# taylorlu/voicepuppet

Hardware: AMD Instinct MI355X
Metric: PixReferNet G+D step frames/sec @256x256 bs=32 (higher is better)
Workload: dtype bf16; 1 GPU; PixReferNet G+D training step (G + 3xD + VGG16-conv3_3 perceptual + TF-Adam x2), 256x256, ngf=ndf=64, global batch 32 = 32 per GPU; global_batch=32, per_gpu_batch=32, parallelism=dp1

## Files before the change

### include/vp_hip.h

```cpp
#ifndef VP_HIP_H_
#define VP_HIP_H_

#include <stddef.h>
#include <stdint.h>

#ifdef __cplusplus
extern "C" {
#endif

enum vp_status { VP_OK = 0, VP_ERR_ARG = -1, VP_ERR_HIP = -2, VP_ERR_WORKSPACE = -3, VP_ERR_STATE = -4 };
enum vp_dtype { VP_F32 = 0, VP_BF16 = 1 };
enum vp_act { VP_ACT_NONE = 0, VP_ACT_LRELU = 1, VP_ACT_RELU = 2, VP_ACT_TANH = 3, VP_ACT_SIGMOID = 4, VP_ACT_RELU6 = 5, VP_ACT_LEAKY = 6 };

int vp_version(void);
const char* vp_last_error(void);

typedef struct vp_pixrefer_desc {
  int batch;
  int height;
  int ngf, ndf;
  int dtype;
  int training;
  float l1_weight;
  float gan_weight;
  int per_sample_bn;
  int streams;
  int d_backward_fork;
  int d_beside_vgg;
} vp_pixrefer_desc;

size_t vp_pixrefer_desc_size(void);

typedef struct vp_pixrefer vp_pixrefer_t;

size_t vp_pixrefer_param_count(const vp_pixrefer_desc* d, int which);
int vp_pixrefer_param_info(const vp_pixrefer_desc* d, int which, int index, char* name, int name_cap,
                           size_t* offset, int* ndim, int64_t shape[4]);

size_t vp_pixrefer_workspace_bytes(const vp_pixrefer_desc* d);
int vp_pixrefer_validate_plan(const vp_pixrefer_desc* d);

int vp_pixrefer_create(const vp_pixrefer_desc* d, void* workspace, size_t workspace_bytes,
                       float* params_g, float* params_d, const float* params_vgg,
                       float* grads_g, float* grads_d, void* stream, vp_pixrefer_t** out);
void vp_pixrefer_destroy(vp_pixrefer_t* h);

int vp_pixrefer_params_changed(vp_pixrefer_t* h);
int vp_pixrefer_optimizer_stepped(vp_pixrefer_t* h);

int vp_pixrefer_forward(vp_pixrefer_t* h, const float* inputs, const float* fg_inputs,
                        const float* targets, const float* masks, void* stream);

int vp_pixrefer_forward_fg3(vp_pixrefer_t* h, const float* inputs, const float* fg_inputs3, const float* targets, void* stream);

int vp_pixrefer_backward(vp_pixrefer_t* h, void* stream);
int vp_pixrefer_backward_update(vp_pixrefer_t* h, float* m_g, float* v_g, float* m_d, float* v_d, int step_t_g, int step_t_d,
                                float lr, float beta1, float beta2, float eps, void* stream);

int vp_pixrefer_backward_d(vp_pixrefer_t* h, void* stream);
int vp_pixrefer_backward_g(vp_pixrefer_t* h, void* stream);
int vp_pixrefer_backward_d_fork(vp_pixrefer_t* h, void* stream);
int vp_pixrefer_backward_d_join(vp_pixrefer_t* h, void* stream);
void* vp_pixrefer_side_stream(vp_pixrefer_t* h);
int vp_reserve_streams(void);
void* vp_host_stream(void);
int vp_pixrefer_use_streams(vp_pixrefer_t* h, int n);
int vp_pixrefer_set_option(vp_pixrefer_t* h, const char* key, int value);
long long vp_pixrefer_counter(vp_pixrefer_t* h, const char* key);
int vp_pixrefer_fetch(vp_pixrefer_t* h, int what, void* dst, void* stream);
int vp_pixrefer_backward_g_stages(void);
int vp_pixrefer_backward_g_stage(vp_pixrefer_t* h, int stage, void* stream);
int vp_pixrefer_update_bucket(vp_pixrefer_t* h, int which, int bucket, float* m, float* v, int step_t, float lr, float beta1,
                              float beta2, float eps, void* stream);

int vp_pixrefer_tensor(vp_pixrefer_t* h, const char* name, void** ptr, int64_t shape[4], int* dtype);

int vp_profile_enable(int on);
size_t vp_profile_collect(char* json, size_t cap);

int vp_pixrefer_pack_frames(const unsigned char* example_frames, const unsigned char* current_frames, const int* crops,
                            int n, int img_size, float* inputs, float* fg_inputs, float* targets, float* masks, void* stream);

int vp_tune(const char* key, int value);
int vp_pixrefer_phase_ms(vp_pixrefer_t* h, float* ms, int cap);
float vp_pixrefer_mark_ms(vp_pixrefer_t* h, int from, int to);

int vp_grad_pack_bf16(const float* src, void* dst_bf16, size_t n, void* stream);
int vp_grad_unpack_bf16(const void* src_bf16, float* dst, size_t n, float scale, void* stream);

int vp_adam_tf(float* params, const float* grads, float* m, float* v, size_t n, int step_t,
               float lr, float beta1, float beta2, float eps, void* stream);

typedef struct vp_conv_desc {
  int kind;
  int n, h, w;
  int cin, cout;
  int ksize, stride, pad;
  int dtype;
  int in_act;
  int out_act;
} vp_conv_desc;

size_t vp_conv_workspace_bytes(const vp_conv_desc* d);
int vp_conv_fwd(const vp_conv_desc* d, const void* x, const float* in_scale, const float* in_shift,
                const float* w, const float* bias, void* y, void* workspace, void* stream);
int vp_conv_bwd_data(const vp_conv_desc* d, const void* dy, const float* w, void* dx, void* workspace, void* stream);
size_t vp_conv3x3_c64_bwd_data_pooled_workspace_bytes(const vp_conv_desc* d);
int vp_conv3x3_c64_bwd_data_pooled(const vp_conv_desc* d, const void* dy_pool, const unsigned char* code, const float* w, const void* ref,
                                   void* dx, void* workspace, int fused, void* stream);
int vp_conv_bwd_weight(const vp_conv_desc* d, const void* x, const float* in_scale, const float* in_shift,
                       const void* dy, float* dw, void* workspace, void* stream);

size_t vp_bn_workspace_bytes(int pixels, int c, int dtype);
int vp_bn_stats(const void* y, int pixels, int c, int dtype, const float* gamma, const float* beta, float eps,
                float* scale, float* shift, float* mean, float* rstd, void* workspace, void* stream);
int vp_bn_bwd(const void* y, const void* dz, void* dy, int pixels, int c, int dtype, const float* gamma,
              const float* mean, const float* rstd, float* dgamma, float* dbeta, void* workspace, void* stream);

typedef struct vp_logmel_desc {
  int sample_rate, num_mel_bins, win_length, hop_step, fft_length;
  float lower_hz, upper_hz;
  int batch, samples;
} vp_logmel_desc;
typedef struct vp_logmel vp_logmel_t;
size_t vp_logmel_workspace_bytes(const vp_logmel_desc* d);
int vp_logmel_frames(const vp_logmel_desc* d);
int vp_logmel_create(const vp_logmel_desc* d, void* workspace, size_t workspace_bytes, void* stream, vp_logmel_t** out);
void vp_logmel_destroy(vp_logmel_t* h);
int vp_logmel_forward(vp_logmel_t* h, const float* pcm, float* out, void* stream);

typedef struct vp_bfmnet_desc {
  int batch;
  int frames;
  int num_mel_bins;
  int trunk_dtype;
} vp_bfmnet_desc;
typedef struct vp_bfmnet vp_bfmnet_t;
size_t vp_bfmnet_param_count(void);
int vp_bfmnet_param_info(int index, char* name, int name_cap, size_t* offset, int* ndim, int64_t shape[4]);
size_t vp_bfmnet_workspace_bytes(const vp_bfmnet_desc* d);
int vp_bfmnet_create(const vp_bfmnet_desc* d, void* workspace, size_t workspace_bytes, const float* params,
                     void* stream, vp_bfmnet_t** out);
// ... 348 lines not shown
```

### voicepuppet_amd/_lib.py

```python
import ctypes
import os

_HERE = os.path.dirname(os.path.abspath(__file__))
LIB_PATH = os.environ.get("VP_LIB", os.path.join(_HERE, "libvp_hip.so"))

VP_F32, VP_BF16 = 0, 1
ACT_NONE, ACT_LRELU, ACT_RELU, ACT_TANH, ACT_SIGMOID = 0, 1, 2, 3, 4


class PixReferDesc(ctypes.Structure):
  _fields_ = [("batch", ctypes.c_int), ("height", ctypes.c_int), ("ngf", ctypes.c_int), ("ndf", ctypes.c_int),
              ("dtype", ctypes.c_int), ("training", ctypes.c_int), ("l1_weight", ctypes.c_float),
              ("gan_weight", ctypes.c_float), ("per_sample_bn", ctypes.c_int),
              ("streams", ctypes.c_int), ("d_backward_fork", ctypes.c_int), ("d_beside_vgg", ctypes.c_int)]


class ConvDesc(ctypes.Structure):
  _fields_ = [("kind", ctypes.c_int), ("n", ctypes.c_int), ("h", ctypes.c_int), ("w", ctypes.c_int),
              ("cin", ctypes.c_int), ("cout", ctypes.c_int), ("ksize", ctypes.c_int), ("stride", ctypes.c_int),
              ("pad", ctypes.c_int), ("dtype", ctypes.c_int), ("in_act", ctypes.c_int), ("out_act", ctypes.c_int)]


class LogMelDesc(ctypes.Structure):
  _fields_ = [("sample_rate", ctypes.c_int), ("num_mel_bins", ctypes.c_int), ("win_length", ctypes.c_int),
              ("hop_step", ctypes.c_int), ("fft_length", ctypes.c_int), ("lower_hz", ctypes.c_float),
              ("upper_hz", ctypes.c_float), ("batch", ctypes.c_int), ("samples", ctypes.c_int)]


class BfmNetDesc(ctypes.Structure):
  _fields_ = [("batch", ctypes.c_int), ("frames", ctypes.c_int), ("num_mel_bins", ctypes.c_int), ("trunk_dtype", ctypes.c_int)]


class BfmStreamDesc(ctypes.Structure):
  _fields_ = [("struct_bytes", ctypes.c_int), ("max_chunk_frames", ctypes.c_int), ("num_mel_bins", ctypes.c_int),
              ("trunk_dtype", ctypes.c_int), ("sample_rate", ctypes.c_int), ("lower_hz", ctypes.c_float), ("upper_hz", ctypes.c_float)]


class BfmStreamGroupDesc(ctypes.Structure):
  _fields_ = [("struct_bytes", ctypes.c_int), ("slots", ctypes.c_int), ("max_chunk_frames", ctypes.c_int), ("num_mel_bins", ctypes.c_int),
# ... 109 lines not shown
                                                 ctypes.c_float, _P]),
    "vp_resize_paste_workspace_bytes": (ctypes.c_size_t, [ctypes.c_int, ctypes.c_int]),
    "vp_resize_paste_u8": (ctypes.c_int, [_P, ctypes.c_int, ctypes.c_int, ctypes.c_int, ctypes.c_int, ctypes.c_int, ctypes.c_int, _P, ctypes.c_int,
                                          ctypes.c_int, ctypes.c_int, ctypes.c_int, _P, _P]),
    "vp_resize_linear_table": (ctypes.c_int, [ctypes.c_int, ctypes.c_int, ctypes.c_int, _P, _P, _P, _P]),
    "vp_mm_workspace_bytes": (ctypes.c_size_t, [ctypes.c_int, ctypes.c_int, ctypes.c_int]),
    "vp_mm_fwd_f32": (ctypes.c_int, [_P, ctypes.c_int, _P, ctypes.c_int, ctypes.c_int, _P, _P, ctypes.c_int, ctypes.c_int, ctypes.c_int, ctypes.c_int, _P, _P]),
    "vp_mm_bwd_data_f32": (ctypes.c_int, [_P, ctypes.c_int, _P, ctypes.c_int, ctypes.c_int, _P, ctypes.c_int, ctypes.c_int, ctypes.c_int, ctypes.c_int,
                                          ctypes.c_int, _P, _P]),
    "vp_mm_bwd_weight_f32": (ctypes.c_int, [_P, ctypes.c_int, _P, ctypes.c_int, _P, ctypes.c_int, ctypes.c_int, ctypes.c_int, ctypes.c_int, _P, _P]),
    "vp_mm_packed_bytes": (ctypes.c_size_t, [ctypes.c_int, ctypes.c_int, ctypes.c_int, ctypes.c_int]),
    "vp_mm_pack_desc_bytes": (ctypes.c_size_t, []),
    "vp_mm_pack_desc": (ctypes.c_int, [ctypes.c_size_t, ctypes.c_int, ctypes.c_int, ctypes.c_int, ctypes.c_int, ctypes.c_int, ctypes.c_int, ctypes.c_size_t, _P]),
    "vp_mm_pack_table": (ctypes.c_int, [_P, ctypes.c_int, _P, _P, _P]),
    "vp_mm_fwd_f32_packed": (ctypes.c_int, [_P, ctypes.c_int, _P, _P, _P, ctypes.c_int, ctypes.c_int, ctypes.c_int, ctypes.c_int, _P, _P]),
    "vp_mm_bwd_data_f32_packed": (ctypes.c_int, [_P, ctypes.c_int, _P, _P, ctypes.c_int, ctypes.c_int, ctypes.c_int, ctypes.c_int, ctypes.c_int, _P, _P]),
    "vp_pixrefer_mark_ms": (ctypes.c_float, [_P, ctypes.c_int, ctypes.c_int]),
    "vp_profile_enable": (ctypes.c_int, [ctypes.c_int]),
    "vp_tune": (ctypes.c_int, [ctypes.c_char_p, ctypes.c_int]),
    "vp_reserve_streams": (ctypes.c_int, []),
    "vp_host_stream": (ctypes.c_void_p, []),
    "vp_pixrefer_pack_frames": (ctypes.c_int, [_P, _P, _P, ctypes.c_int, ctypes.c_int, _P, _P, _P, _P, _P]),
    "vp_profile_collect": (ctypes.c_size_t, [ctypes.c_char_p, ctypes.c_size_t]),
    "vp_pixrefer_tensor": (ctypes.c_int, [_P, ctypes.c_char_p, ctypes.POINTER(_P), ctypes.POINTER(ctypes.c_int64),
                                          ctypes.POINTER(ctypes.c_int)]),
    "vp_adam_tf": (ctypes.c_int, [_P, _P, _P, _P, ctypes.c_size_t, ctypes.c_int, ctypes.c_float, ctypes.c_float,
                                  ctypes.c_float, ctypes.c_float, _P]),
    "vp_conv_workspace_bytes": (ctypes.c_size_t, [ctypes.POINTER(ConvDesc)]),
    "vp_conv_fwd": (ctypes.c_int, [ctypes.POINTER(ConvDesc), _P, _P, _P, _P, _P, _P, _P, _P]),
    "vp_conv_bwd_data": (ctypes.c_int, [ctypes.POINTER(ConvDesc), _P, _P, _P, _P, _P]),
    "vp_conv_bwd_weight": (ctypes.c_int, [ctypes.POINTER(ConvDesc), _P, _P, _P, _P, _P, _P, _P]),
    "vp_conv3x3_c64_bwd_data_pooled_workspace_bytes": (ctypes.c_size_t, [ctypes.POINTER(ConvDesc)]),
    "vp_conv3x3_c64_bwd_data_pooled": (ctypes.c_int, [ctypes.POINTER(ConvDesc), _P, _P, _P, _P, _P, _P, ctypes.c_int, _P]),
    "vp_bn_workspace_bytes": (ctypes.c_size_t, [ctypes.c_int, ctypes.c_int, ctypes.c_int]),
    "vp_bn_stats": (ctypes.c_int, [_P, ctypes.c_int, ctypes.c_int, ctypes.c_int, _P, _P, ctypes.c_float, _P, _P, _P, _P, _P, _P]),
    "vp_logmel_workspace_bytes": (ctypes.c_size_t, [ctypes.POINTER(LogMelDesc)]),
    "vp_logmel_frames": (ctypes.c_int, [ctypes.POINTER(LogMelDesc)]),
    "vp_logmel_create": (ctypes.c_int, [ctypes.POINTER(LogMelDesc), _P, ctypes.c_size_t, _P, ctypes.POINTER(_P)]),
    "vp_logmel_destroy": (None, [_P]),
    "vp_logmel_forward": (ctypes.c_int, [_P, _P, _P, _P]),
    "vp_bfmnet_param_count": (ctypes.c_size_t, []),
    "vp_bfmnet_param_info": (ctypes.c_int, [ctypes.c_int, ctypes.c_char_p, ctypes.c_int, ctypes.POINTER(ctypes.c_size_t),
                                            ctypes.POINTER(ctypes.c_int), ctypes.POINTER(ctypes.c_int64)]),
    "vp_bfmnet_workspace_bytes": (ctypes.c_size_t, [ctypes.POINTER(BfmNetDesc)]),
    "vp_bfmnet_create": (ctypes.c_int, [ctypes.POINTER(BfmNetDesc), _P, ctypes.c_size_t, _P, _P, ctypes.POINTER(_P)]),
    "vp_bfmnet_destroy": (None, [_P]),
    "vp_bfmnet_params_changed": (ctypes.c_int, [_P]),
    "vp_bfmnet_forward": (ctypes.c_int, [_P, _P, _P, _P, _P, _P]),
    "vp_bfmnet_set_decoder_dropout": (ctypes.c_int, [_P, _P, _P]),
    "vp_bfmnet_tensor": (ctypes.c_int, [_P, ctypes.c_char_p, ctypes.POINTER(_P), ctypes.POINTER(ctypes.c_int64)]),
    "vp_bfmstream_desc_size": (ctypes.c_size_t, []),
    "vp_bfmstream_context": (ctypes.c_int, [ctypes.POINTER(BfmStreamDesc)] + [ctypes.POINTER(ctypes.c_int)] * 5),
    "vp_bfmstream_frames_after": (ctypes.c_longlong, [ctypes.POINTER(BfmStreamDesc), ctypes.c_longlong, ctypes.c_int]),
    "vp_bfmstream_workspace_bytes": (ctypes.c_size_t, [ctypes.POINTER(BfmStreamDesc)]),
    "vp_bfmstream_create": (ctypes.c_int, [ctypes.POINTER(BfmStreamDesc), _P, ctypes.c_size_t, _P, _P, ctypes.POINTER(_P)]),
    "vp_bfmstream_destroy": (None, [_P]),
    "vp_bfmstream_params_changed": (ctypes.c_int, [_P]),
    "vp_bfmstream_reset": (ctypes.c_int, [_P, _P]),
    "vp_bfmstream_ready": (ctypes.c_int, [_P, ctypes.c_longlong]),
    "vp_bfmstream_ready_finish": (ctypes.c_int, [_P]),
    "vp_bfmstream_push": (ctypes.c_int, [_P, _P, ctypes.c_longlong, _P, _P, _P]),
    "vp_bfmstream_finish": (ctypes.c_int, [_P, _P, _P, _P]),
    "vp_bfmstream_tensor": (ctypes.c_int, [_P, ctypes.c_char_p, ctypes.POINTER(_P), ctypes.POINTER(ctypes.c_int64)]),
    "vp_bfmstream_group_desc_size": (ctypes.c_size_t, []),
    "vp_puppet_desc_size": (ctypes.c_size_t, []),
    "vp_puppet_workspace_bytes": (ctypes.c_size_t, [ctypes.POINTER(PuppetDesc)]),
# ... 208 lines not shown
```

### voicepuppet_amd/csrc/conv_args.h

```cpp
#pragma once
#include <stddef.h>
#include <stdint.h>

namespace vp {

struct TapTable {
  int8_t dh[16];
  int8_t dw[16];
};

struct PixSrc {
  const void* ptr[2];
  int C[2];
  const float* aff_a[2];
  const float* aff_b[2];
  int act;
  int group_n;
};

enum ConvKernel {
  CK_IGEMM = 0,
  CK_PATCH,
  CK_PATCH2,
  CK_SMALLP,
// ... 34 lines not shown
  int out_act;
  const void* ref;
  const float* ref_a;
  const float* ref_b;
  int ref_act, ref_group_n, accumulate;
  int split_c;
  void* Y2;
  const void* ref2;
  int accumulate2;
  int y2_f32;
  int splitk;
  float* partial;
  int vec_epi;
  int fastk;
  int rowperm;
  int xcd_remap;
  double* bn_part;
  int bn_tpg, bn_nchunk;
  const void* bst_y;
  const void* bst_y2;
  double* bn_part2;
  double* colsum_part;
  const void* zeros;
  int kern, p_kw, p_dhf, p_dhs, p_dwf, p_dws;
  void* xa_lrelu;
  void* xa_relu;
  void* pool_out;
  int pool_only;
  unsigned char* pool_code;
  int pool_src;
  unsigned* sp_cnt;
  unsigned short sp_mask[4];
  int sp_npt, sp_lcpt;
};

struct WgradArgs {
  PixSrc g;
  int Gc, log2Gc;
  int gc_mask;
  int Hgin, Wgin;
  PixSrc d;
  int Dc;
  int N, Hb, Wb;
  int s, ntaps;
  TapTable taps;
  int Mpad, Dpad;
  int splitk;
  float* partial;
  float* dW;
  int Greal, Dreal, accumulate;
  const void* zeros;
  int lw, lh;
  int fastw;
  int xcd_remap;
  int fast_tr;
};

struct Cout1Args {
  const void* dy;
  int ld_dy;
  const float* w;
  const void* ref;
  int ref_act;
  const void* y;
  double* part;
  void* dx;
// ... 9 lines not shown
```

### voicepuppet_amd/csrc/conv_c64.hip

```cpp
#include "conv_ops.h"
#include "igemm_device.h"
#include "launch.h"
#include "patch_device.h"

#ifndef C64_LA
#define C64_LA 2
#endif
#ifndef C64_ABL
#define C64_ABL 0
#endif

namespace vp {

namespace {
constexpr int TH = 4, TW = 16, PW = TW + 2, PH = TH + 2;
constexpr int NPATCH = PW * PH;
constexpr int PPAD = 128;
constexpr int PBUFB = PPAD * 64;
}

__device__ __forceinline__ unsigned pk_max_i16(unsigned x, unsigned y) {
  unsigned r;
  asm("v_pk_max_i16 %0, %1, %2" : "=v"(r) : "v"(x), "v"(y));
  return r;
}
__device__ __forceinline__ unsigned pk_min_u16(unsigned x, unsigned y) {
  unsigned r;
  asm("v_pk_min_u16 %0, %1, %2" : "=v"(r) : "v"(x), "v"(y));
  return r;
}
__device__ __forceinline__ unsigned pk_mul_lo_u16(unsigned x, unsigned y) {
  unsigned r;
  asm("v_pk_mul_lo_u16 %0, %1, %2" : "=v"(r) : "v"(x), "v"(y));
  return r;
}
__device__ __forceinline__ unsigned pk_sub_u16(unsigned x, unsigned y) {
  unsigned r;
  asm("v_pk_sub_u16 %0, %1, %2" : "=v"(r) : "v"(x), "v"(y));
  return r;
}
__device__ __forceinline__ unsigned pk_add_u16(unsigned x, unsigned y) {
  unsigned r;
  asm("v_pk_add_u16 %0, %1, %2" : "=v"(r) : "v"(x), "v"(y));
  return r;
}
__device__ __forceinline__ unsigned pk_max_u16(unsigned x, unsigned y) {
  unsigned r;
  asm("v_pk_max_u16 %0, %1, %2" : "=v"(r) : "v"(x), "v"(y));
  return r;
}
__device__ __forceinline__ unsigned pk_gt_relu(unsigned x, unsigned y) {
  unsigned r;
  asm("v_pk_lshrrev_b16 %0, %1, %2" : "=v"(r) : "v"(0x000F000Fu), "v"(pk_sub_u16(x, y)));
  return r;
}
__device__ __forceinline__ unsigned pk_ashr15_i16(unsigned x) {
  unsigned r;
  asm("v_pk_ashrrev_i16 %0, %1, %2" : "=v"(r) : "v"(0x000F000Fu), "v"(x));
  return r;
}
__device__ __forceinline__ void lds_wr128(int addr, u32x4 v) {
  asm volatile("ds_write_b128 %0, %1\n\ts_nop 1" ::"v"(addr), "v"(v) : "memory");
}
__device__ __forceinline__ unsigned dpp_xor1(unsigned v) {
  return (unsigned)__builtin_amdgcn_update_dpp(0, (int)v, 0xB1, 0xF, 0xF, true);
}

template <int NCH, int TPW, int NW, bool REF, bool RELU, bool POOL, bool STORE, bool CODE = false, bool PSRC = false>
__global__ __launch_bounds__(NW * 64, 2) void conv_c64_kernel(const IgemmArgs a, const int ntiles) {
  static_assert(!POOL || (RELU && !REF), "the packed max pool compares relu outputs");
  static_assert(!CODE || (POOL && !STORE), "pool codes stand in for the full-resolution store");
  static_assert(!PSRC || (REF && NW % NCH == 0 && PH % (NW / NCH) == 0), "pooled source: backward-data, whole waves per channel chunk");
  static_assert((NCH == 2 && TPW == 2) || (NCH == 4 && TPW == 1), "36 NCH TPW <= 144 weight registers");
  constexpr int JP = PPAD / (16 * NW);
  constexpr int CW = 16 * TPW;
  constexpr int COUT = CW * NW, CIN = 32 * NCH;
  constexpr int CB = COUT * 2;
  constexpr int BUFB = NCH * PBUFB;
  constexpr int KS = 9 * NCH;
  static_assert(PPAD % (16 * NW) == 0, "whole DMA rounds per wave");
  constexpr int QH = TH / 2 + 2, QW = TW / 2 + 2, NQ = QH * QW;
  constexpr int SGB = NQ * 64, SCB = NQ * 32, SCODE = NCH * SGB;
  constexpr int NSG = NCH * NQ * 4 / 64;
  constexpr int JS = ((NCH * (SGB + SCB) + 1023) / 1024 + NW - 1) / NW;
  constexpr int STGB = JS * NW * 1024;
  static_assert(!PSRC || (2 * STGB <= BUFB && NCH * NQ * 4 % 64 == 0), "the staging buffers take the second patch buffer's place");
  extern __shared__ __attribute__((aligned(16))) char smem[];
  const int tid = threadIdx.x, lane = tid & 63;
  const int wave = __builtin_amdgcn_readfirstlane(tid >> 6);
  const int fi = lane & 15, fg = lane >> 4;
  const bool flip = a.p_dhs < 0;
  const int dh0 = flip ? a.p_dhf - 2 : a.p_dhf, dw0 = flip ? a.p_dwf - 2 : a.p_dwf;

  uint4 W[KS][TPW];
  {
    const bf16* wp = reinterpret_cast<const bf16*>(a.Wp);
#pragma unroll
    for (int U = 0; U < KS; ++U) {
      const int cc = U / 9, u = U % 9;
      const int tap = flip ? 8 - u : u;
      const size_t chunk_row0 = (size_t)(tap * NCH + cc) * a.wp_rows;
#pragma unroll
      for (int t = 0; t < TPW; ++t) {
        const uint4 w = *reinterpret_cast<const uint4*>(wp + (chunk_row0 + (TPW * wave + t) * 16 + fi) * 32 + fg * 8);
        W[U][t] = (fg & 1) ? make_uint4(w.z, w.w, w.x, w.y) : w;
      }
// ... 13 lines not shown
  }
  int ppy[JP], ppx[JP], prel[JP];
#pragma unroll
  for (int j = 0; j < JP; ++j) {
    const int pp = (wave + NW * j) * 16 + (lane >> 2);
    ppy[j] = pp < NPATCH ? pp / PW : 1 << 20;
    ppx[j] = pp % PW;
    prel[j] = pp < NPATCH ? (ppy[j] * a.Win + ppx[j]) * (CIN * 2) + (((lane & 3) ^ ((ppx[j] >> 1) & 3)) * 8) * (int)sizeof(bf16) : 0;
  }

  const int Hq = a.Hin >> 1, Wq = a.Win >> 1;
  int sqy[JS], sqx[JS], srel[JS];
  if constexpr (PSRC) {
#pragma unroll
    for (int j = 0; j < JS; ++j) {
      const bool g = wave + NW * j < NSG;
      const int v = (wave + NW * j - (g ? 0 : NSG)) * 64 + lane;
      const int upc = g ? NQ * 4 : NQ * 2;
      const int c = v / upc, q = (v % upc) >> (g ? 2 : 1), piece = v & (g ? 3 : 1);
      sqy[j] = c < NCH ? q / QW : 1 << 20;
      sqx[j] = q % QW;
      srel[j] = c < NCH ? ((q / QW) * Wq + sqx[j]) * (g ? CIN * 2 : CIN) + c * (g ? 64 : 32) + piece * 16 : 0;
    }
  }

  __amdgpu_buffer_rsrc_t rsX = make_rsrc(a.x.ptr[0], PSRC ? (unsigned)((size_t)a.N * Hq * Wq * CIN * sizeof(bf16))
                                                          : (unsigned)((size_t)a.N * a.Hin * a.Win * CIN * sizeof(bf16)));
  __amdgpu_buffer_rsrc_t rsC = make_rsrc(PSRC ? (const void*)a.pool_code : a.x.ptr[0], (unsigned)((size_t)a.N * Hq * Wq * CIN));
  const int tiles_x = a.Wg / TW, tpi = tiles_x * (a.Hg / TH);
  const bf16* refp = reinterpret_cast<const bf16*>(a.ref);
  bf16* Yp = reinterpret_cast<bf16*>(a.Y);
  bf16* Pp = reinterpret_cast<bf16*>(a.pool_out);
  constexpr int NSTY = TH * 16 * CB / 1024 / NW;
  constexpr int NST = (STORE ? NSTY : 0) + (POOL ? TH / 2 : 0) + (CODE ? TH / 2 : 0);

  const int G = gridDim.x;
  int bt = blockIdx.x;
  if ((G & 7) == 0) bt = (bt & 7) * (G >> 3) + (bt >> 3);

  auto issue_patch = [&](int t, int buf) {
    const int n = t / tpi, rem = t - n * tpi;
    const int y0 = (rem / tiles_x) * TH, x0 = (rem % tiles_x) * TW;
    const int base = ((n * a.Hin + y0 + dh0) * a.Win + x0 + dw0) * CIN * (int)sizeof(bf16);
#pragma unroll
    for (int j = 0; j < JP; ++j) {
      const int ih = y0 + dh0 + ppy[j], iw = x0 + dw0 + ppx[j];
      const bool ok = (unsigned)ih < (unsigned)a.Hin && (unsigned)iw < (unsigned)a.Win;
      const unsigned vo = ok ? (unsigned)(base + prel[j]) : DMA_OOB;
      uint4* l0 = reinterpret_cast<uint4*>(smem + buf * BUFB) + (wave + NW * j) * 64;
#pragma unroll
      for (int c = 0; c < NCH; ++c) dma16_buf(rsX, vo, (unsigned)(c * 64), l0 + c * (PBUFB / 16));
    }
  };

  auto issue_stage = [&](int t, int sb) {
    const int n = t / tpi, rem = t - n * tpi;
    const int qy0 = (rem / tiles_x) * (TH / 2) - 1, qx0 = (rem % tiles_x) * (TW / 2) - 1;
    const int pix0 = (n * Hq + qy0) * Wq + qx0;
#pragma unroll
    for (int j = 0; j < JS; ++j) {
      const bool g = wave + NW * j < NSG;
      const bool ok = (unsigned)(qy0 + sqy[j]) < (unsigned)Hq && (unsigned)(qx0 + sqx[j]) < (unsigned)Wq;
      const unsigned vo = ok ? (unsigned)(pix0 * (g ? CIN * 2 : CIN) + srel[j]) : DMA_OOB;
      uint4* l0 = reinterpret_cast<uint4*>(smem + BUFB + sb * STGB) + (wave + NW * j) * 64;
      if (g) dma16_buf(rsX, vo, 0u, l0);
      else dma16_buf(rsC, vo, 0u, l0);
    }
// ... 2 lines not shown
  int ex_src = 0, ex_cod = 0, ex_dst = 0, ex_k = 0, ee_src = 0, ee_cod = 0, ee_dst = 0, ee_k = 0;
  const int ec = wave / WPC, er0 = (wave % WPC) * RPW;
  if constexpr (PSRC) {
    const int p = lane & 3;
    {
      const int px = lane >> 2, qx = (px + 1) >> 1;
      ex_src = BUFB + ec * SGB + (qx * 4 + p) * 16;
      ex_cod = BUFB + SCODE + ec * SCB + qx * 32 + p * 8;
      ex_dst = ec * PBUFB + (px << 6) + (((p ^ (px >> 1)) & 3) << 4);
      ex_k = (1 + ((px + 1) & 1)) * 0x00010001;
    }
    {
      const int e = lane >> 2, py = (e >> 1) < PH ? (e >> 1) : PH - 1, px = TW + (e & 1);
      const int q = ((py + 1) >> 1) * QW + ((px + 1) >> 1);
      ee_src = BUFB + ec * SGB + (q * 4 + p) * 16;
      ee_cod = BUFB + SCODE + ec * SCB + q * 32 + p * 8;
      ee_dst = ec * PBUFB + ((py * PW + px) << 6) + (((p ^ (px >> 1)) & 3) << 4);
      ee_k = (1 + 2 * ((py + 1) & 1) + ((px + 1) & 1)) * 0x00010001;
    }
  }

  if constexpr (PSRC) { if (bt < ntiles) issue_stage(bt, 0); }
  else { if (bt < ntiles) issue_patch(bt, 0); }
  int it = 0;
  for (int t = bt; t < ntiles; t += G, ++it) {
    const int buf = it & 1;
    if (it == 0) wait_vm<0>();
    else wait_vm<NST>();
    __builtin_amdgcn_s_barrier();
    asm volatile("" ::: "memory");
    const int n = t / tpi, rem = t - n * tpi;
    const int y0 = (rem / tiles_x) * TH, x0 = (rem % tiles_x) * TW;
    const size_t off00 = ((size_t)(n * a.Hof + y0) * a.Wof + x0 + fi) * COUT + c0;
    unsigned rz[TH][NV / 2];
    if constexpr (REF) {
#pragma unroll
      for (int r = 0; r < TH; ++r) {
        if constexpr (NV == 8) {
          const uint4 z = *reinterpret_cast<const uint4*>(refp + off00 + (size_t)r * a.Wof * COUT);
          rz[r][0] = z.x; rz[r][1] = z.y; rz[r][NV / 2 - 2] = z.z; rz[r][NV / 2 - 1] = z.w;
        } else {
          const uint2 z = *reinterpret_cast<const uint2*>(refp + off00 + (size_t)r * a.Wof * COUT);
          rz[r][0] = z.x; rz[r][1] = z.y;
        }
      }
    }
    if constexpr (PSRC) {
      if (t + G < ntiles && (!(C64_ABL & 1) || it < 1)) issue_stage(t + G, buf ^ 1);
      const int sb = buf * STGB;
      u32x4 eg[2];
      u32x2 ew[2];
      auto erd = [&](auto jc) {
        constexpr int j = decltype(jc)::value;
        const int qo = j < RPW ? ((er0 + j + 1) >> 1) * QW : 0;
        eg[j & 1] = lds_rd128<0>((j < RPW ? ex_src + qo * 64 : ee_src) + sb);
        ew[j & 1] = lds_rd64<0>((j < RPW ? ex_cod + qo * 32 : ee_cod) + sb);
      };
      erd(std::integral_constant<int, 0>{});
      static_steps([&](auto jc) {
        constexpr int j = decltype(jc)::value;
        if constexpr (j < RPW) erd(std::integral_constant<int, j + 1>{});
        asm volatile("s_waitcnt lgkmcnt(%0)" ::"n"((j > 0 ? 1 : 0) + (j < RPW ? 2 : 0)) : "memory");
        asm volatile("" : "+v"(eg[j & 1]), "+v"(ew[j & 1]));
        const unsigned k = j < RPW ? (unsigned)ex_k + (unsigned)((er0 + j + 1) & 1) * 0x00020002u : (unsigned)ee_k;
        u32x4 o;
#pragma unroll
        for (int d = 0; d < 4; ++d) {
          const unsigned cw = d < 2 ? ew[j & 1].x : ew[j & 1].y;
// ... 20 lines not shown
    constexpr int LA = C64_LA, NS = LA + 1, NSTEP = NCH * 3 * PH;
    u32x4 rb[NS];
    auto rd = [&](auto sc) {
      constexpr int S = decltype(sc)::value, cc = S / (3 * PH), pc = (S / PH) % 3, R = S % PH;
      if constexpr ((C64_ABL & 8) != 0) { if (S >= NS) return; }
      rb[S % NS] = lds_rd128<cc * PBUFB + R * PW * 64>(tb[pc]);
    };
    static_steps([&](auto sc) { rd(sc); }, std::make_integer_sequence<int, LA>{});
    static_steps([&](auto sc) {
      constexpr int S = decltype(sc)::value, cc = S / (3 * PH), pc = (S / PH) % 3, R = S % PH;
      if constexpr (S + LA < NSTEP) rd(std::integral_constant<int, S + LA>{});
      constexpr int AHEAD = (NSTEP - 1 - S < LA ? NSTEP - 1 - S : LA);
      asm volatile("s_waitcnt lgkmcnt(%0)" ::"n"(AHEAD) : "memory");
      asm volatile("" : "+v"(rb[S % NS]));
      const uint4 fb = make_uint4(rb[S % NS].x, rb[S % NS].y, rb[S % NS].z, rb[S % NS].w);
      static_steps([&](auto ri) {
        constexpr int r = R - 2 + decltype(ri)::value;
        if constexpr (r >= 0 && r < TH) {
          constexpr int U = cc * 9 + (R - r) * 3 + pc;
#pragma unroll
          for (int tt = 0; tt < TPW; ++tt) { if (!(C64_ABL & 4)) acc[r][tt] = mma16<bf16>(W[U][tt], fb, acc[r][tt]); else acc[r][tt][0] += __uint_as_float(fb.x ^ W[U][tt].x); }
        }
      }, std::make_integer_sequence<int, 3>{});
      __builtin_amdgcn_sched_barrier(0);
    }, std::make_integer_sequence<int, NSTEP>{});

    unsigned pk[TH][NV / 2];
#pragma unroll
    for (int r = 0; r < TH; ++r) {
#pragma unroll
      for (int e = 0; e < NV / 2; ++e) {
        unsigned o = Elem<bf16>::pack2(acc[r][(2 * e) >> 2][(2 * e) & 3], acc[r][(2 * e + 1) >> 2][(2 * e + 1) & 3]);
        if constexpr (RELU) o = pk_max_i16(o, 0u);
        if constexpr (REF) o = pk_mul_lo_u16(o, pk_min_u16(pk_max_i16(rz[r][e], 0u), 0x00010001u));
        pk[r][e] = o;
      }
    }
    if constexpr (STORE) {
      char* stg = smem + 2 * BUFB;
      constexpr int SPP = CB / 16;
#pragma unroll
      for (int r = 0; r < TH; ++r) {
        char* q = stg + (r * 16 + fi) * CB + ((((c0 * 2) >> 4) ^ (fi & 7)) << 4) + ((c0 * 2) & 15);
        if constexpr (NV == 8) *reinterpret_cast<uint4*>(q) = make_uint4(pk[r][0], pk[r][1], pk[r][NV / 2 - 2], pk[r][NV / 2 - 1]);
        else *reinterpret_cast<uint2*>(q) = make_uint2(pk[r][0], pk[r][1]);
      }
      asm volatile("s_waitcnt lgkmcnt(0)" ::: "memory");
      __builtin_amdgcn_s_barrier();
      asm volatile("" ::: "memory");
      if (!(C64_ABL & 2) || pk[0][0] == 0x12345u) {
#pragma unroll
        for (int j = 0; j < NSTY; ++j) {
          constexpr int PPI = 64 / SPP;
          const int g = wave * NSTY + j;
          const int pi = g * PPI + lane / SPP, row = pi >> 4, px = pi & 15, sl = lane % SPP;
          const uint4 o = *reinterpret_cast<const uint4*>(stg + (row * 16 + px) * CB + ((sl ^ (px & 7)) << 4));
          unsigned* yp = reinterpret_cast<unsigned*>(Yp + ((size_t)(n * a.Hof + y0 + row) * a.Wof + x0 + px) * COUT + sl * 8);
          __builtin_nontemporal_store(o.x, yp); __builtin_nontemporal_store(o.y, yp + 1);
          __builtin_nontemporal_store(o.z, yp + 2); __builtin_nontemporal_store(o.w, yp + 3);
        }
      }
    }
    if constexpr (POOL) {
#pragma unroll
      for (int q = 0; q < TH; q += 2) {
        unsigned m[NV / 2], cd[NV / 2];
#pragma unroll
        for (int e = 0; e < NV / 2; ++e) {
          if constexpr (CODE) {
            const unsigned v0 = pk[q][e], v1 = dpp_xor1(v0), v2 = pk[q + 1][e], v3 = dpp_xor1(v2);
            const unsigned g1 = pk_gt_relu(v0, v1), m1 = pk_max_i16(v0, v1);
            const unsigned g2 = pk_gt_relu(m1, v2), m2 = pk_max_i16(m1, v2);
            const unsigned g3 = pk_gt_relu(m2, v3);
            m[e] = pk_max_i16(m2, v3);
            const unsigned best = pk_max_u16(pk_max_u16(g1, pk_add_u16(g2, g2)), pk_mul_lo_u16(g3, 0x00030003u));
            cd[e] = pk_mul_lo_u16(pk_min_u16(m[e], 0x00010001u), pk_add_u16(best, 0x00010001u));
          } else {
            m[e] = pk_max_i16(pk[q][e], pk[q + 1][e]);
            m[e] = pk_max_i16(m[e], dpp_xor1(m[e]));
          }
        }
        if (!(fi & 1)) {
          const size_t po = ((size_t)(n * (a.Hg >> 1) + ((y0 + q) >> 1)) * (a.Wg >> 1) + ((x0 + fi) >> 1)) * COUT + c0;
          if constexpr (NV == 8) *reinterpret_cast<uint4*>(Pp + po) = make_uint4(m[0], m[1], m[NV / 2 - 2], m[NV / 2 - 1]);
          else *reinterpret_cast<uint2*>(Pp + po) = make_uint2(m[0], m[1]);
          if constexpr (CODE) {
            const unsigned w0 = __builtin_amdgcn_perm(cd[1], cd[0], 0x06040200u);
            if constexpr (NV == 8) *reinterpret_cast<uint2*>(a.pool_code + po) = make_uint2(w0, __builtin_amdgcn_perm(cd[NV / 2 - 1], cd[NV / 2 - 2], 0x06040200u));
            else *reinterpret_cast<unsigned*>(a.pool_code + po) = w0;
          }
        }
      }
    }
  }
}

bool conv_c64_eligible(const IgemmArgs& a, int is_bf16) {
  if (!is_bf16 || conv_staging(a.kern) != CK_PATCH || !patch3_eligible(a, 1)) return false;
  if ((a.Cin != 64 && a.Cin != 128) || a.x.C[0] != a.Cin || (a.Cout != 64 && a.Cout != 128)) return false;
  if (a.CoutPad != a.Cout || a.ldY != a.Cout || !a.rowperm || a.splitk != 1) return false;
  if (a.Hg % TH || a.Wg % TW || a.Hin != a.Hg || a.Win != a.Wg || a.Hof != a.Hg || a.Wof != a.Wg) return false;
  if ((a.out_act != ACT_NONE && a.out_act != ACT_RELU) || (a.ref && (a.ref_act != ACT_RELU || a.out_act != ACT_NONE || a.pool_out))) return false;
  if (a.pool_out && (a.out_act != ACT_RELU || (a.Hg & 1))) return false;
  if (a.pool_only && !a.pool_out) return false;
  if (a.pool_code && !a.pool_only && !a.pool_src) return false;
  if (a.pool_src && (!a.ref || !a.pool_code || a.Cin != a.Cout)) return false;
  if (a.bn_part || a.accumulate || a.y_f32 || a.ref_a || a.split_c || a.x.aff_a[0] || a.x.act != ACT_NONE) return false;
  if (a.p_dhs != a.p_dws || a.p_dhf != a.p_dwf || a.p_dhf != (a.p_dhs > 0 ? -1 : 1)) return false;
  return (size_t)a.N * a.Hin * a.Win * a.Cin * 2 < 0x70000000ull;
}

template <int NCH, int TPW, int NW>
static hipError_t launch_c64_t(const IgemmArgs& a, hipStream_t st) {
  const int ntiles = a.N * (a.Hg / TH) * (a.Wg / TW);
  void (*kern)(const IgemmArgs, const int);
  if (a.ref && a.pool_src) {
    if constexpr (16 * TPW * NW == 32 * NCH) kern = conv_c64_kernel<NCH, TPW, NW, true, false, false, true, false, true>;
    else return hipErrorInvalidValue;
  } else if (a.ref) kern = conv_c64_kernel<NCH, TPW, NW, true, false, false, true>;
  else if (a.pool_out && a.pool_code) kern = conv_c64_kernel<NCH, TPW, NW, false, true, true, false, true>;
  else if (a.pool_out) kern = a.pool_only ? conv_c64_kernel<NCH, TPW, NW, false, true, true, false> : conv_c64_kernel<NCH, TPW, NW, false, true, true, true>;
  else kern = a.out_act == ACT_RELU ? conv_c64_kernel<NCH, TPW, NW, false, true, false, true> : conv_c64_kernel<NCH, TPW, NW, false, false, false, true>;
  const int smem = 2 * NCH * PBUFB + TH * 16 * (16 * TPW * NW * 2);
  const int blocks = 256 * (8 / NW);
  (void)hipFuncSetAttribute((const void*)kern, hipFuncAttributeMaxDynamicSharedMemorySize, smem);
  hipLaunchKernelGGL(kern, dim3(ntiles < blocks ? ntiles : blocks), dim3(NW * 64), smem, st, a, ntiles);
  return hipGetLastError();
}

hipError_t launch_conv_c64(const IgemmArgs& a, hipStream_t st) {
  if (a.Cin == 64) return a.Cout == 64 ? launch_c64_t<2, 2, 2>(a, st) : launch_c64_t<2, 2, 4>(a, st);
  return a.Cout == 64 ? launch_c64_t<4, 1, 4>(a, st) : launch_c64_t<4, 1, 8>(a, st);
}

}
```

### voicepuppet_amd/csrc/conv_kernels.hip

```cpp
#include <stdio.h>
#include <stdlib.h>
#include <string.h>

#include <string>
#include <vector>

#include "conv_args.h"
#include "conv_ops.h"
#include "errors.h"
#include "igemm_device.h"
#include "smallp_args.h"
#include "launch.h"
#include "vp_common.h"

#ifndef VP_RING
#define VP_RING 3
#endif
#ifndef VP_REGB_EPI_BYTES
#define VP_REGB_EPI_BYTES (36 * 1024)
#endif
#ifndef VP_ABLATE
#define VP_ABLATE 0
#endif

// ... 1061 lines not shown
        const size_t se = (size_t)(BP / NPE) * (BC * 4 + 16) + (BP / NPE) * 8;
        if (se > sm) sm = se;
        g_prof_family = "ws";
        if (bst && b.split_c) hipLaunchKernelGGL((igemm_ws_kernel<T, WC, WP, TC, TP, NSTW, 2, true>), grid, dim3((NW + 4) * 64), sm, st, b);
        else if (bst) hipLaunchKernelGGL((igemm_ws_kernel<T, WC, WP, TC, TP, NSTW, 2>), grid, dim3((NW + 4) * 64), sm, st, b);
        else if (b.bn_part) hipLaunchKernelGGL((igemm_ws_kernel<T, WC, WP, TC, TP, NSTW, 1>), grid, dim3((NW + 4) * 64), sm, st, b);
        else if (b.split_c) hipLaunchKernelGGL((igemm_ws_kernel<T, WC, WP, TC, TP, NSTW, 0, true>), grid, dim3((NW + 4) * 64), sm, st, b);
        else hipLaunchKernelGGL((igemm_ws_kernel<T, WC, WP, TC, TP, NSTW, 0>), grid, dim3((NW + 4) * 64), sm, st, b);
        return hipGetLastError();
      }
    }
    g_prof_family = "dma";
    if (bst && !b.vec_epi) return hipErrorInvalidValue;
    if (bst && b.split_c) hipLaunchKernelGGL((igemm_dma_kernel<T, WC, WP, TC, TP, true, 2, true>), grid, dim3(NW * 64), smem, st, b);
    else if (bst) hipLaunchKernelGGL((igemm_dma_kernel<T, WC, WP, TC, TP, true, 2>), grid, dim3(NW * 64), smem, st, b);
    else if (b.vec_epi && b.bn_part) hipLaunchKernelGGL((igemm_dma_kernel<T, WC, WP, TC, TP, true, 1>), grid, dim3(NW * 64), smem, st, b);
    else if (b.vec_epi && b.split_c) hipLaunchKernelGGL((igemm_dma_kernel<T, WC, WP, TC, TP, true, 0, true>), grid, dim3(NW * 64), smem, st, b);
    else if (b.vec_epi) hipLaunchKernelGGL((igemm_dma_kernel<T, WC, WP, TC, TP, true>), grid, dim3(NW * 64), smem, st, b);
    else if (b.split_c) hipLaunchKernelGGL((igemm_dma_kernel<T, WC, WP, TC, TP, false, 0, true>), grid, dim3(NW * 64), smem, st, b);
    else hipLaunchKernelGGL((igemm_dma_kernel<T, WC, WP, TC, TP, false>), grid, dim3(NW * 64), smem, st, b);
    return hipGetLastError();
  }
  g_prof_family = "reg";
  if (a.bst_y || a.bst_y2) return hipErrorInvalidValue;
  if (a.split_c) return hipErrorInvalidValue;
  if constexpr (NW == 4) hipLaunchKernelGGL((igemm_kernel<T, WC, WP, TC, TP>), grid, dim3(256), 2 * 4 * (BC + BP) * 16 + 64, st, a);
  else return hipErrorInvalidValue;
  return hipGetLastError();
}


bool conv_kernel_ok(const IgemmArgs& a, int is_bf16) {
  if (a.pool_src && a.kern != CK_C64) return false;
  switch (a.kern) {
    case CK_IGEMM: case CK_PATCH: case CK_PATCH2: case CK_SMALLP: return true;
    case CK_S2C64: return conv_s2c64_eligible(a, is_bf16);
    case CK_CIN8: return conv_cin8_eligible(a, is_bf16);
    case CK_COUT8: return conv_cout8_eligible(a, is_bf16);
    case CK_DCOUT8: return conv_dcout8_eligible(a, is_bf16);
    case CK_COUT4: return conv_cout4_eligible(a, is_bf16);
    case CK_C64: return conv_c64_eligible(a, is_bf16);
    case CK_PATCH3: return patch3_eligible(a, is_bf16);
    case CK_PATCH4: return patch4_eligible(a, is_bf16);
    case CK_DC256: return conv_dc256_eligible(a, is_bf16);
    case CK_DC64: return conv_dc64_eligible(a, is_bf16);
    default: return false;
  }
}

const char* conv_kernel_name(int kern) {
  static const char* const names[] = {"igemm", "patch", "patch2", "smallp", "s2c64", "cin8", "cout8", "dcout8", "cout4", "c64", "patch3", "patch4",
                                      "dc256", "dc64"};
  return kern >= 0 && kern <= CK_DC64 ? names[kern] : "?";
}

template <typename T> static hipError_t launch_igemm_t(const IgemmArgs& a, int cfg, hipStream_t st) {
  constexpr bool bf = sizeof(T) == 2;
  if (!conv_kernel_ok(a, bf)) {
    set_err("launch_igemm: the arguments are outside the preconditions of the plan's kernel %s (%s, %d x %d x %d -> %d channels)",
            conv_kernel_name(a.kern), bf ? "bf16" : "f32", a.N, a.Hg, a.Wg, a.Cout);
    return hipErrorInvalidValue;
  }
  hipError_t e;
  int pbc, pbp;
  igemm_tile(cfg, &pbc, &pbp);
  const double Pn = (double)a.N * a.Hg * a.Wg * a.nclass;
// ... 184 lines not shown
```

### voicepuppet_amd/csrc/conv_ops.h

```cpp
#pragma once
#include <stdlib.h>
#include <string.h>

#include "launch.h"

namespace vp {

struct ConvGeomX : ConvGeom {
  int CoutT;
};

inline ConvGeomX make_geom(int kind, int ks, int stride, int pad, int N, int Hin, int Win, int Cin, int Cin_real, int Cout) {
  ConvGeomX g;
  g.kind = kind; g.ks = ks; g.stride = stride; g.pad = pad;
  g.N = N; g.Hin = Hin; g.Win = Win;
  if (kind == 0) { g.Hout = (Hin + 2 * pad - ks) / stride + 1; g.Wout = (Win + 2 * pad - ks) / stride + 1; }
  else { g.Hout = 2 * Hin; g.Wout = 2 * Win; }
  g.Cin = Cin; g.Cin_real = Cin_real; g.Cout = Cout;
  g.CoutT = Cout < 8 ? 8 : Cout;
  return g;
}

inline int kc_elems(int is_bf16) { return is_bf16 ? 32 : 16; }

// ... 8 lines not shown
    if (rows % 256 == 0 && P >= 256 * 256 && Kpad >= 4096) return 7;
    if (rows % 128 == 0 && P >= 256 * 512) return 6;
    if (rows % 128 == 0) return 0;
    if (rows % 64 == 0) return 1;
    if (rows <= 16) return 2;
    return rows > 64 ? 0 : 1;
  }
  if (rows <= 64) return 5;
  return P > 16 ? 3 : 4;
}

constexpr int IGEMM_SPLITK_TARGET_DEFAULT = 64;
inline int& igemm_splitk_target_knob() { static int v = IGEMM_SPLITK_TARGET_DEFAULT; return v; }
inline int pick_igemm_splitk(int blocks, int nchunk) {
  const int target = igemm_splitk_target_knob();
  const int cap = plan_misc_knob(1);
  const int minchunk = plan_misc_knob(2);
  if (blocks >= 256 || blocks >= target) return 1;
  int s = (target + blocks - 1) / blocks;
  if (s > nchunk / minchunk) s = nchunk / minchunk;
  if (s > cap) s = cap;
  return s < 1 ? 1 : s;
}

inline void set_single_src(PixSrc& x, const void* p, int C, const float* a, const float* b, int act, int group_n) {
  x.ptr[0] = p; x.ptr[1] = nullptr; x.C[0] = C; x.C[1] = 0;
  x.aff_a[0] = a; x.aff_b[0] = b; x.aff_a[1] = nullptr; x.aff_b[1] = nullptr;
  x.act = act; x.group_n = group_n > 0 ? group_n : (1 << 30);
}

struct LaunchForm {
  bool bias = false, ref = false, xa_lrelu = false, xa_relu = false, x_affine = false;
  bool stats = false;
  int x_act = 0, ref_act = 0;
};

struct IgemmPlan {
  IgemmArgs a;
  int cfg;
  LaunchForm form;
  PackDesc pack;
  size_t pack_elems;
  size_t partial_bytes;
};

struct IgemmPin { int cfg, splitk; };

inline void finish_igemm(IgemmPlan& p, int rows, int is_bf16, const IgemmPin* pin = nullptr) {
  IgemmArgs& a = p.a;
  const int P = a.N * a.Hg * a.Wg;
  a.Kpad = round_up(a.ntaps * a.Cin, kc_elems(is_bf16));
  p.cfg = pick_igemm_cfg(rows, P, a.Kpad);
  if (!is_bf16 && a.ntaps == 1 && p.cfg == 0) {
    const long long b128 = (long long)((P + 127) / 128) * (rows / 128), b64 = 2 * b128;
    if (((b64 + 255) / 256) * 64 < ((b128 + 255) / 256) * 128) p.cfg = 1;
  }
  if (pin) p.cfg = pin->cfg;
  int bc, bp;
  igemm_tile(p.cfg, &bc, &bp);
  a.CoutPad = round_up(rows, bc);
  if (a.ntaps == 1) { a.log2Cin = 30; a.cin_mask = 0x3fffffff; }
  else { a.log2Cin = ilog2(a.Cin); a.cin_mask = a.Cin - 1; }
  const int blocks = ((P + bp - 1) / bp) * (a.CoutPad / bc) * a.nclass;
  a.splitk = pin ? pin->splitk : pick_igemm_splitk(blocks, a.Kpad / kc_elems(is_bf16));
  p.partial_bytes = a.splitk > 1 ? (size_t)a.nclass * a.splitk * P * a.CoutPad * sizeof(float) : 0;
  {
    const bool tc4 = p.cfg == 0 || p.cfg == 1 || p.cfg == 6 || p.cfg == 7 || p.cfg == 8 || p.cfg == 9;
    a.rowperm = (tc4 && rows % 64 == 0) ? 1 : 0;
    p.pack.perm = a.rowperm;
  }
  a.wp_rows = round_up(rows, 128);
  p.pack.rows_pad = a.wp_rows;
  p.pack.Kpad = a.Kpad;
  p.pack.kc = kc_elems(is_bf16);
  p.pack_elems = (size_t)a.nclass * a.wp_rows * a.Kpad;
}

inline int& patch_tiles_knob() { static int v = 7; return v; }
inline int& patch_small_knob() { static int v = 3; return v; }
inline int& patch_longk_knob() { static int v = 1; return v; }
inline int& patch3_knob() { static int v = 1; return v; }
inline int& wgrad_big_knob() { static int v = 1; return v; }
inline int& patch4_knob() { static int v = 1; return v; }
inline int& c64_knob() { static int v = 1; return v; }
inline int& pool_bwd_fused_knob() { static int v = 1; return v; }
inline int& cout1_knob() { static int v = 256; return v; }
inline int& wgrad1_rows_knob() { static int v = 512; return v; }
inline int& dc64_knob() { static int v = 1; return v; }
inline int& s2c64_knob() { static int v = 512; return v; }
inline int& s2c64_pair_knob() { static int v = 1; return v; }
constexpr int PATCH_MIN_BLOCKS_DEFAULT = 192;
inline int& patch_minblk_knob() { static int v = PATCH_MIN_BLOCKS_DEFAULT; return v; }

inline void patch_tile_hw(int bp, int* th, int* tw) { *th = bp == 128 ? 8 : 16; *tw = bp == 512 ? 32 : 16; }
inline int patch_tile_pixels(int bc) {
  const int k = patch_small_knob();
  if (bc == 256) return (k & 2) ? 128 : 256;
  return (k & 1) ? 256 : 512;
}

inline int patch_tile_rows(int rows, int on) {
  if ((on & 1) && rows % 256 == 0) return 256;
  if ((on & 2) && rows % 128 == 0) return 128;
  if ((on & 4) && rows % 64 == 0) return 64;
  return 0;
}

inline bool plan_patch_eligible(const IgemmPlan& p, int rows, int is_bf16, bool single_src, bool any_grid = false) {
  const int on = patch_tiles_knob();
  const int minblk = any_grid ? 0 : patch_minblk_knob();
  const IgemmArgs& a = p.a;
  const int kc = kc_elems(is_bf16);
  if (!on || !single_src || a.nclass != 1 || a.sh != 1 || a.sw != 1 || a.os != 1 || a.ntaps < 9 || a.Cin % kc || a.Cin < kc) return false;
  if (rows % 64 || a.Cout % 8 || a.ldY % 8 || a.Hg < 16 || a.Wg < 16 || a.Hof != a.Hg || a.Wof != a.Wg) return false;
  const bool p4 = patch4_knob() && is_bf16 && a.ntaps == 16 && rows % 128 == 0;
  if (!p4 && patch_longk_knob() && rows >= 512 && rows % 256 == 0 && a.ntaps * a.Cin >= 4096 && (long long)a.N * a.Hg * a.Wg >= 256 * 256) return false;
  const int bc = p4 ? 128 : patch_tile_rows(rows, on);
  if (!bc) return false;
// ... 110 lines not shown
  if (s > 64) s = 64;
  if (s < 1) s = 1;
  a.splitk = s;
  p.partial_bytes = s > 1 ? (size_t)s * tiles * PT * 32 * sizeof(float) : 0;
}

inline bool plan_s2c64_eligible(const IgemmPlan& p, int rows, int is_bf16, int c0, int c1) {
  const IgemmArgs& a = p.a;
  if (s2c64_knob() <= 0 || !is_bf16 || a.nclass != 1 || a.ntaps != 16 || a.os != 1 || a.sh != 2 || a.sw != 2) return false;
  if ((rows != 128 && rows != 256) || a.Cout != rows || a.ldY != 128 || a.Cin != 64 || c0 != 64 || c1 != 0 || a.Kpad != 1024) return false;
  if (a.Hg % 4 || a.Wg % 16 || a.Hin != 2 * a.Hg || a.Win != 2 * a.Wg || a.Hof != a.Hg || a.Wof != a.Wg) return false;
  for (int t = 0; t < 16; ++t)
    if (a.taps[0].dh[t] != (t >> 2) - 1 || a.taps[0].dw[t] != (t & 3) - 1) return false;
  if (a.N * (a.Hg / 4) * (a.Wg / 16) < s2c64_knob()) return false;
  return (size_t)a.N * a.Hin * a.Win * 64 * 2 < 0x70000000ull;
}
inline void plan_make_s2c64(IgemmPlan& p) {
  IgemmArgs& a = p.a;
  a.kern = CK_S2C64;
  p.cfg = 0;
  a.CoutPad = a.Cout; a.wp_rows = a.Cout; p.pack.rows_pad = a.Cout;
  p.pack_elems = (size_t)a.wp_rows * a.Kpad;
  a.splitk = 1; p.partial_bytes = 0;
  a.rowperm = 1; p.pack.perm = 1; p.pack.kswap = 0;
}

inline IgemmArgs launch_view(const IgemmPlan& p, const LaunchForm& f) {
  static char set[16] = {};
  IgemmArgs v = p.a;
  v.Y = set; v.zeros = set;
  if (v.split_c) v.Y2 = set;
  if (f.bias) v.bias = (const float*)set;
  if (f.ref) { v.ref = set; v.ref_act = f.ref_act; if (v.split_c) v.ref2 = set; }
  if (f.xa_lrelu) v.xa_lrelu = set;
  if (f.xa_relu) v.xa_relu = set;
  if (f.x_affine) v.x.aff_a[0] = (const float*)set;
  v.x.act = f.x_act;
  if (f.stats) v.bn_part = (double*)set;
  return v;
}

inline int pick_conv_kernel(const IgemmArgs& v, int is_bf16) {
  const int fam = conv_staging(v.kern);
  if (fam == CK_SMALLP || fam == CK_S2C64) return fam;
  if (is_bf16) {
    if (conv_cin8_eligible(v, 1)) return CK_CIN8;
    if (conv_cout8_eligible(v, 1)) return CK_COUT8;
    if (conv_dcout8_eligible(v, 1)) return CK_DCOUT8;
    if (conv_cout4_eligible(v, 1)) return CK_COUT4;
    if (c64_knob() && conv_c64_eligible(v, 1)) return CK_C64;
    if (dc64_knob() && conv_dc256_eligible(v, 1)) return CK_DC256;
    if (dc64_knob() && conv_dc64_eligible(v, 1)) return CK_DC64;
    if (patch4_knob() && patch4_eligible(v, 1)) return CK_PATCH4;
  }
  if (fam == CK_PATCH && patch3_knob() && patch3_eligible(v, is_bf16)) return CK_PATCH3;
  return fam;
}

enum { FAM_SMALLP = 1, FAM_PATCH = 2, FAM_PATCH2 = 4, FAM_S2C64 = 8, FAM_ALL = 15 };

inline void plan_kernel(IgemmPlan& p, int rows, int is_bf16, int c0, int c1, unsigned fams, const LaunchForm& f, bool any_grid = false) {
  if ((fams & FAM_SMALLP) && plan_smallp_eligible(p, rows, is_bf16, c0, c1)) plan_make_smallp(p, rows, is_bf16);
  else if ((fams & FAM_PATCH) && plan_patch_eligible(p, rows, is_bf16, c1 == 0 && c0 == p.a.Cin, any_grid)) plan_make_patch(p, rows, is_bf16);
  else if ((fams & FAM_PATCH2) && plan_patch2_eligible(p, rows, is_bf16, c0, c1)) plan_make_patch2(p, rows, is_bf16);
  else if ((fams & FAM_S2C64) && plan_s2c64_eligible(p, rows, is_bf16, c0, c1)) plan_make_s2c64(p);
  p.form = f;
// ... 155 lines not shown
```

### voicepuppet_amd/csrc/conv_thin.hip

```cpp
#include "conv_ops.h"
#include "igemm_device.h"
#include "launch.h"
#include "thin_device.h"
#include "vp_common.h"

namespace vp {

template <int S, int OUTS>
__global__ __launch_bounds__(256) void conv_cin8_kernel(const IgemmArgs a, int lgW, int lgH) {
  const int lane = threadIdx.x & 63;
  const int i = lane & 15, g = lane >> 4;
  const int P = a.N << (lgW + lgH);
  const int ntile = P >> 4;
  const int wave_global = blockIdx.x * 4 + (threadIdx.x >> 6), nwave = gridDim.x * 4;

  __shared__ uint4 wfrag[S * 4 * 64];
  __shared__ uint4 otile[4 * 16 * 144 / 16];
  constexpr bool ACTS = (OUTS & 6) != 0;
  {
    const bf16* wp = reinterpret_cast<const bf16*>(a.Wp);
    for (int idx = threadIdx.x; idx < S * 4 * 64; idx += 256) {
      const int l = idx & 63, t = (idx >> 6) & 3, s = idx >> 8;
      const int row = a.rowperm ? t * 16 + (l & 15) : (t >> 1) * 32 + 8 * ((l & 15) >> 2) + (t & 1) * 4 + (l & 3);
      wfrag[idx] = *reinterpret_cast<const uint4*>(wp + ((size_t)s * a.wp_rows + row) * 32 + (l >> 4) * 8);
    }
    __syncthreads();
  }
  float bias[16];
#pragma unroll
  for (int e = 0; e < 16; ++e) bias[e] = a.bias ? a.bias[(e >> 3) * 32 + 8 * g + (e & 7)] : 0.f;
  const float act_floor = a.out_act == ACT_RELU ? 0.f : -__builtin_inff();
  int tdh[S], tdw[S];
  bool tok[S];
#pragma unroll
  for (int s = 0; s < S; ++s) {
    const int tap = 4 * s + g;
    tok[s] = tap < a.ntaps;
    int dh = 0, dw = 0;
#pragma unroll
    for (int t = 0; t < 16; ++t) if (t == tap) { dh = a.taps[0].dh[t]; dw = a.taps[0].dw[t]; }
    tdh[s] = dh; tdw[s] = dw;
// ... 9 lines not shown
    const int ow = p & ((1 << lgW) - 1), oh = (p >> lgW) & ((1 << lgH) - 1), n = p >> (lgW + lgH);
    const int bh = oh * a.sh, bw = ow * a.sw;
#pragma unroll
    for (int s = 0; s < S; ++s) {
      const int ih = bh + tdh[s], iw = bw + tdw[s];
      const bool ok = tok[s] && (unsigned)ih < (unsigned)a.Hin && (unsigned)iw < (unsigned)a.Win;
      const unsigned off = ok ? (unsigned)(((n * a.Hin + ih) * a.Win + iw) * 16) : DMA_OOB;
      const u32x4 v = __builtin_amdgcn_raw_buffer_load_b128(rsX, (int)off, 0, 0);
      fb[s] = make_uint4(v.x, v.y, v.z, v.w);
    }
  };
  auto finish_tile = [&](int tile_, const uint4 (&fb)[S]) {
    const int tile = tile_ < tile_last ? tile_ : tile_last;
    f32x4 acc[4];
#pragma unroll
    for (int t = 0; t < 4; ++t) acc[t] = (f32x4){0.f, 0.f, 0.f, 0.f};
    int wl = lane;
    asm volatile("" : "+v"(wl));
#pragma unroll
    for (int s = 0; s < S; ++s)
#pragma unroll
      for (int t = 0; t < 4; ++t) acc[t] = mma16<bf16>(wfrag[(s * 4 + t) * 64 + wl], fb[s], acc[t]);
    const int p = tile * 16 + i;
    float lo[8], hi[8];
#pragma unroll
    for (int t = 0; t < 4; ++t)
#pragma unroll
      for (int e = 0; e < 4; ++e) {
        const float x = fmaxf(acc[t][e] + bias[4 * t + e], act_floor);
        if (t < 2) lo[4 * t + e] = x; else hi[4 * (t - 2) + e] = x;
      }
    const uint4 plo = Elem<bf16>::pack(lo), phi = Elem<bf16>::pack(hi);
    char* tb = reinterpret_cast<char*>(otile) + (threadIdx.x >> 6) * (16 * 144);
    auto store_run = [&](void* dst, const uint4& v0, const uint4& v1) {
      *reinterpret_cast<uint4*>(tb + i * 144 + g * 16) = v0;
      *reinterpret_cast<uint4*>(tb + i * 144 + 64 + g * 16) = v1;
      __builtin_amdgcn_s_waitcnt(0xc07f);
      __builtin_amdgcn_wave_barrier();
      const uint4 q0 = *reinterpret_cast<const uint4*>(tb + (lane >> 3) * 144 + (lane & 7) * 16);
      const uint4 q1 = *reinterpret_cast<const uint4*>(tb + (8 + (lane >> 3)) * 144 + (lane & 7) * 16);
      bf16* yt = reinterpret_cast<bf16*>(dst) + (size_t)tile * 16 * 64;
      reinterpret_cast<uint4*>(yt)[lane] = q0;
      reinterpret_cast<uint4*>(yt)[64 + lane] = q1;
      __builtin_amdgcn_wave_barrier();
    };
    if constexpr (OUTS & 1) store_run(a.Y, plo, phi);
    if constexpr (ACTS) {
      float rl[8], rh[8];
      Elem<bf16>::unpack(plo, rl);
      Elem<bf16>::unpack(phi, rh);
      if constexpr (OUTS & 2) {
        float t0[8], t1[8];
#pragma unroll
        for (int e = 0; e < 8; ++e) { t0[e] = act_apply(ACT_LRELU, rl[e]); t1[e] = act_apply(ACT_LRELU, rh[e]); }
        store_run(a.xa_lrelu, Elem<bf16>::pack(t0), Elem<bf16>::pack(t1));
      }
      if constexpr (OUTS & 4) {
        float t0[8], t1[8];
#pragma unroll
        for (int e = 0; e < 8; ++e) { t0[e] = act_apply(ACT_RELU, rl[e]); t1[e] = act_apply(ACT_RELU, rh[e]); }
        store_run(a.xa_relu, Elem<bf16>::pack(t0), Elem<bf16>::pack(t1));
      }
    }
  };

  uint4 fb0[S], fb1[S], fb2[S], fb3[S];
  int tile = wave_global;
  load_tile(tile, fb0);
  load_tile(tile + nwave, fb1);
  load_tile(tile + 2 * nwave, fb2);
  for (int trip = (my_n + 3) / 4; trip > 0; --trip) {
    load_tile(tile + 3 * nwave, fb3);
    finish_tile(tile, fb0);
    load_tile(tile + 4 * nwave, fb0);
    finish_tile(tile + nwave, fb1);
    load_tile(tile + 5 * nwave, fb1);
    finish_tile(tile + 2 * nwave, fb2);
    load_tile(tile + 6 * nwave, fb2);
    finish_tile(tile + 3 * nwave, fb3);
    tile += 4 * nwave;
  }
}

template <int SPT, int HALVED>
__global__ __launch_bounds__(256) void deconv_cout4_tile_kernel(const IgemmArgs a, int lgW, int lgH) {
  typedef ThinHalo<SPT * 32> H;
  constexpr int S = 9 * SPT, CIN = H::CIN, PPP = H::PPP, PIXB = H::PIXB, TPX = H::TPX, NPIECE = H::NPIECE, NJ = H::NJ;
  extern __shared__ __attribute__((aligned(16))) char smem[];
  uint4* wfrag = reinterpret_cast<uint4*>(smem);
  char* stage = smem + thin_weight_image_bytes<SPT, 1>;
  const int lane = threadIdx.x & 63, wv = threadIdx.x >> 6;
  const int i = lane & 15, g = lane >> 4;
  {
    const bf16* wp = reinterpret_cast<const bf16*>(a.Wp);
// ... 244 lines not shown
    for (int u = 0; u < 9; ++u) {
      const char* px = stage + ((wv + u / 3) * 18 + i + u % 3) * PIXB + g * 16;
#pragma unroll
      for (int k = 0; k < SPT; ++k) {
        const uint4 b = *reinterpret_cast<const uint4*>(px + k * 64);
        acc0 = mma16<bf16>(wfrag[(u * SPT + k) * 64 + wl], b, acc0);
        acc1 = mma16<bf16>(wfrag[(S + u * SPT + k) * 64 + wl], b, acc1);
      }
    }
    const int tl = tile < tile_last ? tile : tile_last;
    const int tc = tl & (tw - 1), tr = (tl >> (lgW - 4)) & (th - 1), n = tl >> (lgW - 4 + lgH - 2);
    const int q = tr * 4 + wv, r = tc * 16 + i;
#pragma unroll
    for (int T = 0; T < 2; ++T) {
      const f32x4 acc = T ? acc1 : acc0;
      float v[8];
#pragma unroll
      for (int e = 0; e < 4; ++e) { v[e] = acc[e]; v[4 + e] = __shfl(acc[e], (lane + 16) & 63); }
      const int cls = 2 * T + (g >> 1);
      const unsigned yo = (g & 1) == 0 ? (unsigned)((((n * a.Hof + 2 * q + (cls >> 1)) * a.Wof + 2 * r + (cls & 1)) * a.ldY) * 2) : DMA_OOB;
      const uint4 pk = Elem<bf16>::pack(v);
      __builtin_amdgcn_raw_buffer_store_b128((u32x4){pk.x, pk.y, pk.z, pk.w}, rsY, (int)yo, 0, 0);
    }
    tile += gridDim.x;
  }
}

bool conv_cin8_eligible(const IgemmArgs& a, int is_bf16) {
  const bool pow2 = (a.Wg & (a.Wg - 1)) == 0 && (a.Hg & (a.Hg - 1)) == 0;
  return is_bf16 && a.zeros && a.Cin == 8 && a.x.C[0] == 8 && a.x.C[1] == 0 && a.Cout == 64 && a.ldY == 64 && a.nclass == 1 && a.splitk == 1 && a.os == 1 &&
         a.Hof == a.Hg && a.Wof == a.Wg && pow2 && !a.ref && !a.accumulate && !a.y_f32 && !a.bn_part && !a.x.aff_a[0] && a.x.act == ACT_NONE &&
         a.ntaps <= 16 && (a.Kpad == 96 || a.Kpad == 128) && (size_t)a.N * a.Hin * a.Win * 16 < 0x70000000ull &&
         (((long long)a.N * a.Hg * a.Wg) & 15) == 0 && (a.out_act == ACT_NONE || a.out_act == ACT_RELU) &&
         (a.Kpad == 128 || !(a.xa_lrelu || a.xa_relu)) && !(a.xa_relu && !a.xa_lrelu);
}

bool conv_cout8_eligible(const IgemmArgs& a, int is_bf16) {
  bool near = a.ntaps == 9;
  for (int t = 0; near && t < 9; ++t) near = a.taps[0].dh[t] >= -1 && a.taps[0].dh[t] <= 1 && a.taps[0].dw[t] >= -1 && a.taps[0].dw[t] <= 1;
  return is_bf16 && near && a.zeros && a.nclass == 1 && a.sh == 1 && a.sw == 1 && a.os == 1 && a.Cin == 64 && a.x.C[0] == 64 && a.x.C[1] == 0 &&
         a.CoutPad == 16 && a.Cout <= 8 && a.ldY == 8 && a.splitk == 1 && !a.rowperm && !a.bn_part && !a.x.aff_a[0] && a.x.act == ACT_NONE &&
         (a.Wg & (a.Wg - 1)) == 0 && (a.Hg & (a.Hg - 1)) == 0 && a.Wg >= 16 && a.Hg >= 4 && a.Hof == a.Hg && a.Wof == a.Wg && a.Hin == a.Hg &&
         a.Win == a.Wg && !a.y_f32 && (size_t)a.N * a.Hin * a.Win * 64 * 2 < 0x70000000ull &&
         !a.bias && a.out_act == ACT_NONE && !a.ref && !a.accumulate && !a.split_c;
}

bool conv_dcout8_eligible(const IgemmArgs& a, int is_bf16) {
  return is_bf16 && a.zeros && a.nclass == 4 && a.os == 2 && a.ntaps == 4 && a.Cin == 64 && a.x.C[0] == 64 && a.x.C[1] == 0 && a.CoutPad == 16 &&
         a.Cout <= 8 && a.ldY == 8 && !a.y_f32 && a.splitk == 1 && !a.rowperm && !a.bn_part && !a.x.aff_a[0] && a.x.act == ACT_NONE &&
         (a.Wg & (a.Wg - 1)) == 0 && (a.Hg & (a.Hg - 1)) == 0 && a.Wg >= 16 && a.Hg >= 4 && a.Hof == 2 * a.Hg && a.Wof == 2 * a.Wg && a.Hin == a.Hg &&
         a.Win == a.Wg && (size_t)a.N * a.Hin * a.Win * 64 * 2 < 0x70000000ull && (size_t)a.N * a.Hof * a.Wof * 8 * 2 < 0x70000000ull &&
         !a.bias && a.out_act == ACT_NONE && !a.ref && !a.accumulate && !a.split_c;
}

bool conv_cout4_eligible(const IgemmArgs& a, int is_bf16) {
  const bool pow2 = (a.Wg & (a.Wg - 1)) == 0 && (a.Hg & (a.Hg - 1)) == 0;
  const int spt = a.Cin / 32;
  return is_bf16 && a.zeros && a.nclass == 4 && a.os == 2 && a.ntaps == 4 && a.Cout == 4 && a.y_f32 && a.ldY == 4 && a.splitk == 1 && pow2 &&
         a.Wg >= 16 && a.Hg >= 4 && a.Cin % 32 == 0 && (spt == 2 || spt == 4) && a.x.C[1] == a.x.C[0] && a.x.C[0] + a.x.C[1] == a.Cin &&
         !a.ref && !a.accumulate && a.out_act == ACT_NONE && !a.x.aff_a[0] && !a.x.aff_a[1] && a.x.act == ACT_NONE && a.Hof == 2 * a.Hg &&
         a.Wof == 2 * a.Wg && (size_t)a.N * a.Hin * a.Win * a.Cin * 2 < 0x70000000ull && (size_t)a.N * a.Hof * a.Wof * 16 < 0x70000000ull;
}

struct ThinGrid { int lgW, lgH, blocks; };
static ThinGrid thin_grid(const IgemmArgs& a, int knob) {
  ThinGrid g{ilog2(a.Wg), ilog2(a.Hg), 0};
  g.blocks = ((a.N << (g.lgW + g.lgH)) + 63) >> 6;
  if (g.blocks > thin_blocks_knob(knob)) g.blocks = thin_blocks_knob(knob);
  return g;
}

template <typename K> static hipError_t launch_thin_tile(K kern, const IgemmArgs& a, int knob, int smem, hipStream_t st) {
  const ThinGrid g = thin_grid(a, knob);
  if (smem > 48 * 1024) (void)hipFuncSetAttribute((const void*)kern, hipFuncAttributeMaxDynamicSharedMemorySize, smem);
  hipLaunchKernelGGL(kern, dim3(g.blocks), dim3(256), (size_t)smem, st, a, g.lgW, g.lgH);
  return hipGetLastError();
}

hipError_t launch_conv_cin8(const IgemmArgs& a, hipStream_t st) {
  const ThinGrid g = thin_grid(a, 3);
  const int outs = (a.Y ? 1 : 0) | (a.xa_lrelu ? 2 : 0) | (a.xa_relu ? 4 : 0);
  void (*kern)(const IgemmArgs, int, int) = nullptr;
  if (a.Kpad == 96) kern = outs == 1 ? conv_cin8_kernel<3, 1> : nullptr;
  else switch (outs) {
    case 1: kern = conv_cin8_kernel<4, 1>; break;
    case 2: kern = conv_cin8_kernel<4, 2>; break;
    case 3: kern = conv_cin8_kernel<4, 3>; break;
    case 6: kern = conv_cin8_kernel<4, 6>; break;
    case 7: kern = conv_cin8_kernel<4, 7>; break;
    default: break;
  }
  if (!kern) return hipErrorInvalidValue;
  hipLaunchKernelGGL(kern, dim3(g.blocks), dim3(256), 0, st, a, g.lgW, g.lgH);
  return hipGetLastError();
}

hipError_t launch_conv_cout8(const IgemmArgs& a, hipStream_t st) {
  return launch_thin_tile(conv3x3_cout8_tile_kernel, a, 0, ThinHalo<64>::LDS_BYTES, st);
}

hipError_t launch_conv_dcout8(const IgemmArgs& a, hipStream_t st) {
  return launch_thin_tile(deconv_cout8_tile_kernel<2>, a, 1, thin_weight_image_bytes<2, 2> + ThinHalo<64>::LDS_BYTES, st);
}

hipError_t launch_conv_cout4(const IgemmArgs& a, hipStream_t st) {
  if (a.Cin == 64) return launch_thin_tile(deconv_cout4_tile_kernel<2, 1>, a, 2, thin_weight_image_bytes<2, 1> + ThinHalo<64>::LDS_BYTES, st);
  return launch_thin_tile(deconv_cout4_tile_kernel<4, 1>, a, 2, thin_weight_image_bytes<4, 1> + ThinHalo<128>::LDS_BYTES, st);
}

}
```

### voicepuppet_amd/csrc/ops_api.hip

```cpp
#include <string.h>

#include <string>

#include "conv_ops.h"
#include "errors.h"
#include "audio_args.h"
#include "launch.h"
#include "vp_common.h"

using namespace vp;

namespace {

bool conv_desc_ok(const vp_conv_desc* d) {
  if (!d || d->n < 1 || d->h < 1 || d->w < 1) return false;
  if (d->cin < 8 || (d->cin & (d->cin - 1))) return false;
  if (d->kind == 1 && (d->ksize != 4 || d->stride != 2 || d->pad != 1)) return false;
  if (d->kind != 0 && d->kind != 1) return false;
  if (d->ksize < 1 || d->ksize > 4 || d->stride < 1 || d->stride > 2) return false;
  if (d->kind == 0 && d->stride == 2 && (d->ksize != 4 || d->pad != 1 || (d->h & 1) || (d->w & 1))) return false;
  return d->dtype == VP_F32 || d->dtype == VP_BF16;
}

ConvGeomX geom_of(const vp_conv_desc* d) {
  return make_geom(d->kind, d->ksize, d->stride, d->pad, d->n, d->h, d->w, d->cin, d->cin, d->cout);
}

size_t align256(size_t v) { return (v + 255) & ~(size_t)255; }

const void* zero_page(char* ws, size_t used, hipStream_t st) {
  char* z = ws + align256(used);
  (void)hipMemsetAsync(z, 0, 256, st);
  return z;
}

}

extern "C" {

int vp_pixrefer_pack_frames(const unsigned char* example_frames, const unsigned char* current_frames, const int* crops,
                            int n, int img_size, float* inputs, float* fg_inputs, float* targets, float* masks, void* stream) {
  if (!example_frames || !current_frames || !crops || !inputs || !fg_inputs || !targets || !masks || n < 1 || img_size < 2) {
    set_err("vp_pixrefer_pack_frames: bad argument");
    return VP_ERR_ARG;
  }
  FramePackArgs a;
  a.ex = example_frames; a.cur = current_frames; a.crops = crops;
  a.inputs = inputs; a.fg_inputs = fg_inputs; a.targets = targets; a.masks = masks;
  a.N = n; a.S = img_size;
  VP_HIP_CHECK(launch_frame_pack(a, (hipStream_t)stream));
  return VP_OK;
}

extern "C" void vp_phase_marks_enable(int on);

int vp_tune(const char* key, int value) {
  if (!key) return VP_ERR_ARG;
  const std::string k(key);
  if (k == "patch_tiles") { patch_tiles_knob() = value; return VP_OK; }
  if (k == "patch_min_blocks") { patch_minblk_knob() = value < 0 ? PATCH_MIN_BLOCKS_DEFAULT : value; return VP_OK; }
  if (k == "patch_small_tiles") { patch_small_knob() = value; return VP_OK; }
  if (k == "patch_long_k_on_256") { patch_longk_knob() = value; return VP_OK; }
  if (k == "wgrad_tr") { wgrad_tr_knob() = value; return VP_OK; }
  if (k == "patch3") { patch3_knob() = value; return VP_OK; }
  if (k == "c64") { c64_knob() = value; return VP_OK; }
  if (k == "dc64") { dc64_knob() = value; return VP_OK; }
  if (k == "pool_bwd_fused") { pool_bwd_fused_knob() = value < 0 || value > 4 ? 1 : value; return VP_OK; }
  if (k == "cout1_wgrad_rows" && value > 0) { wgrad1_rows_knob() = value; return VP_OK; }
  if (k == "cout1_bwd") { cout1_knob() = value < 0 ? 256 : value; return VP_OK; }
  if (k == "s2c64") { s2c64_knob() = value; return VP_OK; }
  if (k == "wgrad_big") { wgrad_big_knob() = value; return VP_OK; }
  if (k == "patch4") { patch4_knob() = value; return VP_OK; }
  if (k == "s2c64_pair") { s2c64_pair_knob() = value; return VP_OK; }
  if (k == "bfm_dwproj") { bfm_dwproj_knob() = value; return VP_OK; }
  if (k == "patch2") { patch2_knob() = value; return VP_OK; }
  if (k == "patch_xcd") { patch_xcd_knob() = value; return VP_OK; }
  if (k == "smallp_max_pixels") { smallp_knob() = value; return VP_OK; }
  if (k == "igemm_splitk_target") { igemm_splitk_target_knob() = value < 0 ? IGEMM_SPLITK_TARGET_DEFAULT : value; return VP_OK; }
  if (k == "wgrad_fixed_x10") { wgrad_cost_knob(0) = value; return VP_OK; }
  if (k == "wgrad_slab_tile_x1000") { wgrad_cost_knob(2) = value < 0 ? 150 : value; return VP_OK; }
  if (k == "wgrad_slab_x100") { wgrad_cost_knob(1) = value; return VP_OK; }
  if (k == "smallp_split_target") { plan_misc_knob(0) = value; return VP_OK; }
  if (k == "igemm_splitk_cap") { plan_misc_knob(1) = value; return VP_OK; }
  if (k == "igemm_splitk_minchunk") { plan_misc_knob(2) = value; return VP_OK; }
  if (k == "wgrad_resident_blocks") { plan_misc_knob(3) = value; return VP_OK; }
  if (k == "igemm_small_grid") { igemm_small_grid_knob() = value; return VP_OK; }
  if (k == "thin_blocks_cout8" && value > 0) { thin_blocks_knob(0) = value; return VP_OK; }
  if (k == "thin_blocks_dcout8" && value > 0) { thin_blocks_knob(1) = value; return VP_OK; }
  if (k == "thin_blocks_cout4" && value > 0) { thin_blocks_knob(2) = value; return VP_OK; }
  if (k == "thin_blocks_cin8" && value > 0) { thin_blocks_knob(3) = value; return VP_OK; }
  if (k == "phase_marks") { vp_phase_marks_enable(value); return VP_OK; }
  set_err("vp_tune: unknown key %s", key);
  return VP_ERR_ARG;
}

static unsigned* smallp_counter_page(char* ws, size_t used, const IgemmArgs& a, hipStream_t st) {
  unsigned* c = (unsigned*)(ws + align256(used) + 256);
  (void)hipMemsetAsync(c, 0, (size_t)smallp_counters(a) * sizeof(unsigned), st);
  return c;
}
// ... 45 lines not shown
  VP_HIP_CHECK(launch_pack_weights_one(p.pack, w, ws, bf, st));
  IgemmArgs a = p.a;
  set_single_src(a.x, x, d->cin, in_scale, in_shift, d->in_act, 0);
  a.Wp = ws;
  a.partial = (float*)(ws + align256(p.pack_elems * es));
  a.Y = y; a.bias = bias;
  a.zeros = zero_page(ws, align256(p.pack_elems * es) + p.partial_bytes, st);
  if (a.kern == CK_SMALLP) a.sp_cnt = smallp_counter_page(ws, align256(p.pack_elems * es) + p.partial_bytes, a, st);
  VP_HIP_CHECK(launch_igemm(a, bf, p.cfg, st));
  return VP_OK;
}

int vp_conv_bwd_data(const vp_conv_desc* d, const void* dy, const float* w, void* dx, void* workspace, void* stream) {
  if (!conv_desc_ok(d) || !dy || !w || !dx || !workspace) { set_err("vp_conv_bwd_data: bad argument"); return VP_ERR_ARG; }
  if (d->cout < 8 || (d->cout & (d->cout - 1))) { set_err("vp_conv_bwd_data: cout must be a power of two >= 8"); return VP_ERR_ARG; }
  const int bf = d->dtype == VP_BF16, es = bf ? 2 : 4;
  hipStream_t st = (hipStream_t)stream;
  const ConvGeomX g = geom_of(d);
  IgemmPlan p = plan_bwd_data(g, 0, 0, d->cin, d->cin, d->cin, bf);
  plan_kernel(p, d->cin, bf, d->cout, 0, FAM_SMALLP | FAM_PATCH | FAM_PATCH2, LaunchForm{});
  char* ws = (char*)workspace;
  VP_HIP_CHECK(launch_pack_weights_one(p.pack, w, ws, bf, st));
  IgemmArgs a = p.a;
  set_single_src(a.x, dy, d->cout, nullptr, nullptr, ACT_NONE, 0);
  a.Wp = ws;
  a.partial = (float*)(ws + align256(p.pack_elems * es));
  a.Y = dx;
  a.zeros = zero_page(ws, align256(p.pack_elems * es) + p.partial_bytes, st);
  if (a.kern == CK_SMALLP) a.sp_cnt = smallp_counter_page(ws, align256(p.pack_elems * es) + p.partial_bytes, a, st);
  VP_HIP_CHECK(launch_igemm(a, bf, p.cfg, st));
  return VP_OK;
}

static bool pooled_desc_ok(const vp_conv_desc* d) {
  return conv_desc_ok(d) && d->kind == 0 && d->ksize == 3 && d->stride == 1 && d->pad == 1 && d->dtype == VP_BF16 && d->cin == d->cout &&
         (d->cin == 64 || d->cin == 128) && d->h % 4 == 0 && d->w % 16 == 0 && d->h >= 16;
}

size_t vp_conv3x3_c64_bwd_data_pooled_workspace_bytes(const vp_conv_desc* d) {
  if (!pooled_desc_ok(d)) return 0;
  return align256(vp_conv_workspace_bytes(d)) + align256((size_t)d->n * d->h * d->w * d->cout * 2) + 256;
}

int vp_conv3x3_c64_bwd_data_pooled(const vp_conv_desc* d, const void* dy_pool, const unsigned char* code, const float* w, const void* ref,
                                   void* dx, void* workspace, int fused, void* stream) {
  if (!pooled_desc_ok(d) || !dy_pool || !code || !w || !ref || !dx || !workspace) { set_err("vp_conv3x3_c64_bwd_data_pooled: bad argument"); return VP_ERR_ARG; }
  hipStream_t st = (hipStream_t)stream;
  const ConvGeomX g = geom_of(d);
  IgemmPlan p = plan_bwd_data(g, 0, 0, d->cin, d->cin, d->cin, 1);
  LaunchForm f;
  f.ref = true; f.ref_act = ACT_RELU;
  plan_kernel(p, d->cin, 1, d->cout, 0, FAM_PATCH, f);
  if (p.a.kern != CK_C64) {
    set_err("vp_conv3x3_c64_bwd_data_pooled: %d x %d x %d x %d is planned on kernel %s, not c64", d->n, d->h, d->w, d->cin, conv_kernel_name(p.a.kern));
    return VP_ERR_ARG;
  }
  char* ws = (char*)workspace;
  VP_HIP_CHECK(launch_pack_weights_one(p.pack, w, ws, 1, st));
  IgemmArgs a = p.a;
  a.Wp = ws;
  a.partial = (float*)(ws + align256(p.pack_elems * 2));
  a.Y = dx;
  a.ref = ref; a.ref_act = ACT_RELU;
  a.zeros = zero_page(ws, align256(p.pack_elems * 2) + p.partial_bytes, st);
  if (fused) {
    set_single_src(a.x, dy_pool, d->cout, nullptr, nullptr, ACT_NONE, 0);
// ... 215 lines not shown
```

### voicepuppet_amd/csrc/plan_pixrefer.hip

```cpp
#include <math.h>
#include <stdio.h>
#include <string.h>

#include <mutex>
#include <string>
#include <utility>
#include <vector>

#include "conv_ops.h"
#include "errors.h"
#include "launch.h"
#include "smallp_args.h"
#include "vp_common.h"

namespace vp {

thread_local char g_err[512] = "";
void set_err(const char* fmt, ...) {
  va_list ap;
  va_start(ap, fmt);
  vsnprintf(g_err, sizeof(g_err), fmt, ap);
  va_end(ap);
}

struct Arena {
  char* base;
  size_t off, cap;
  std::vector<std::pair<size_t, size_t>>* track = nullptr;
  void* alloc(size_t bytes) {
    off = (off + 255) & ~(size_t)255;
    void* p = base ? base + off : nullptr;
    if (track) track->push_back({off, bytes});
    off += bytes;
    return p;
  }
};

struct BnBuf {
  float *a, *b, *mu, *rstd, *c1, *c2, *c1g, *c2g;
  double *pb, *pbg;
};

struct Tens {
  std::string name;
  void* y = nullptr;
  void* dz = nullptr;
  int N = 0, H = 0, W = 0, C = 0;
  bool is_f32 = false;
  bool has_bn = false;
  bool is_input = false;
  bool dz_written = false;
  void* dz2 = nullptr;
  bool dz2_written = false;
  void* xa[3] = {nullptr, nullptr, nullptr};
  bool need_act[3] = {false, false, false};
  BnBuf bn{};
  int producer = -1;
  int n_bwd_consumers = 0;
  int dz_writes = 0;
  bool bn_bwd_done = false;
  bool hi = false;
  void* dz32 = nullptr;
  double* cs_part = nullptr;
  int cs_chunks = 0;
  int pb_cap = 0, pbg_cap = 0;
  int bst_chunks = 0, bst_chunks_g = 0;
  size_t elems() const { return (size_t)N * H * W * C; }
};

struct Layer {
  std::string scope;
  ConvGeomX g;
  int src[2] = {-1, -1};
  int nsrc = 1;
  int in_act = ACT_NONE;
  int out_act = ACT_NONE;
  int out = -1;
  bool has_bn = false;
  size_t w_off = 0, b_off = 0, gamma_off = 0, beta_off = 0;
  size_t pk_fwd = 0, pk_bwd[2] = {0, 0}, pk_bwd_alt[2] = {0, 0};
  bool need_bwd[2] = {false, false};
  IgemmPlan fwd, bwd[2], bwd_alt[2];
  IgemmPlan bwd_pair;
  size_t pk_bwd_pair = 0;
  bool has_pair = false;
  IgemmPlan fwd_half;
  size_t pk_fwd_half = 0;
// ... 14 lines not shown
struct Net {
  std::vector<Tens> t;
  std::vector<Layer> l;
  std::vector<ParamInfo> manifest;
  size_t nparams = 0;
  int batch = 0, groups = 1;
  float* params = nullptr;
  float* grads = nullptr;
  char* packed = nullptr;
  size_t packed_elems = 0;
  std::vector<PackDesc> descs;
  PackDesc* d_descs = nullptr;
  unsigned* sp_cnt = nullptr;
  size_t sp_cnt_n = 0;
};

}

using namespace vp;

struct vp_pixrefer {
  vp_pixrefer_desc d;
  int bf16, es;
  Net G, D, V;
  void *gin, *gfg, *din, *vin;
  float *y4, *o4, *outputs, *outputs_fg, *logits, *predict, *losses;
  void *dl_d, *dl_g, *d_din, *d_vin, *dy4, *df3;
  void *vpool1, *vpool2, *d_vpool1, *d_vpool2;
  unsigned char* vpool_code[2];
  bool pool_codes_written;
  bool pool_fuse_ok[2];
  bool pool_bwd_fused;
  bool pool_dz_stale[2];
  double *comp_partial, *perc_partial, *bn_partial;
  char* scratch;
  char* scratch2;
  double* bn_partial2;
  char* scratch3;
  double* bn_partial3;
  char* scratch4;
  double* bn_partial4;
  hipStream_t side, branch;
  hipStream_t branch2;
  hipEvent_t ev_b2join;
  bool use_b2;
  hipEvent_t ev_fork, ev_join, ev_bfork, ev_bjoin;
  hipEvent_t ev_upd_b, ev_upd_m;
  bool overlap, forked;
  int bst_count;
  int bst_on;
  int vgg_fork_layer;
  bool store_first_raw;
  bool ov_on;
  int dfork_point;
  bool dsplit_on;
  hipEvent_t mark[64];
  int nmark;
  bool marks_made;
  int dfork_pending;
  void* zeros;
  size_t scratch_bytes;
  int n_comp, n_perc;
  struct { bool active, d_done; float *m_g, *v_g, *m_d, *v_d; float lr_t_g, lr_t_d, beta1, beta2, eps; } upd;
  int upd_mask;
  bool params_dirty;
  bool vgg_dirty;
// ... 262 lines not shown
      for (int s = 0; s < L.nsrc; ++s) {
        if (!L.need_bwd[s]) continue;
        Tens& ts = n.t[L.src[s]];
        cap(ts, L.bwd[s], n.batch, n.groups, ts.pb_cap);
        if (alt_batch > 0) cap(ts, L.bwd_alt[s], alt_batch, 1, ts.pbg_cap);
        if (L.has_pair) cap(ts, L.bwd_pair, n.batch, n.groups, ts.pb_cap);
        if (L.tapgemm && bf16 && ts.has_bn && !ts.hi && L.g.ks == 4 && L.g.stride == 1 && L.g.Cin == 512) {
          if (ts.pb_cap < 256) ts.pb_cap = 256;
          if (alt_batch > 0 && ts.pbg_cap < 256) ts.pbg_cap = 256;
        }
      }
    }
  for (size_t i = 0; i < n.l.size(); ++i) n.l[i].desc1 = i + 1 < n.l.size() ? n.l[i + 1].desc0 : n.descs.size();
  for (Tens& t : n.t) t.n_bwd_consumers = 0;
  n.sp_cnt_n = 0;
  for (Layer& L : n.l) {
    if (L.fwd.a.kern == CK_SMALLP) n.sp_cnt_n += smallp_counters(L.fwd.a);
    for (int s = 0; s < L.nsrc && training; ++s) {
      if (!L.need_bwd[s]) continue;
      n.t[L.src[s]].n_bwd_consumers++;
      if (L.bwd[s].a.kern == CK_SMALLP) n.sp_cnt_n += smallp_counters(L.bwd[s].a);
    }
    if (training && L.has_pair && L.bwd_pair.a.kern == CK_SMALLP) n.sp_cnt_n += smallp_counters(L.bwd_pair.a);
  }
}

static void carve_net(Net& n, Arena& ar, int es, bool training) {
  for (Tens& t : n.t) {
    if (t.name == "decoder_1" || t.name == "layer_5") {
      continue;
    }
    if (!t.is_input) t.y = ar.alloc(t.elems() * (t.hi ? sizeof(float) : (size_t)es));
    for (int k = 1; k < 3; ++k) if (t.need_act[k]) t.xa[k] = ar.alloc(t.elems() * es);
    if (t.has_bn) {
      const size_t gc = (size_t)n.groups * t.C * sizeof(float);
      t.bn.a = (float*)ar.alloc(gc); t.bn.b = (float*)ar.alloc(gc);
      t.bn.mu = (float*)ar.alloc(gc); t.bn.rstd = (float*)ar.alloc(gc);
      t.bn.c1 = (float*)ar.alloc(gc); t.bn.c2 = (float*)ar.alloc(gc);
      t.bn.c1g = (float*)ar.alloc(gc); t.bn.c2g = (float*)ar.alloc(gc);
      t.bn.pb = (training && t.pb_cap) ? (double*)ar.alloc((size_t)n.groups * t.pb_cap * 2 * t.C * sizeof(double)) : nullptr;
      t.bn.pbg = (training && t.pbg_cap) ? (double*)ar.alloc((size_t)t.pbg_cap * 2 * t.C * sizeof(double)) : nullptr;
    }
  }
  for (Layer& L : n.l) {
    if (!L.tapgemm) continue;
    const size_t q = (size_t)L.g.N * L.g.Hin * L.g.Win * 16;
    L.tap_S = (float*)ar.alloc(q * sizeof(float));
    L.tap_dyS = ar.alloc(q * es);
  }
  n.packed = (char*)ar.alloc(n.packed_elems * es);
  n.d_descs = (PackDesc*)ar.alloc(n.descs.size() * sizeof(PackDesc));
  n.sp_cnt = (unsigned*)ar.alloc((n.sp_cnt_n + 1) * sizeof(unsigned));
  {
    unsigned* c = n.sp_cnt;
    for (Layer& L : n.l) {
      if (L.fwd.a.kern == CK_SMALLP) { L.sp_cnt_fwd = c; c += c ? smallp_counters(L.fwd.a) : 0; }
      for (int s = 0; s < L.nsrc && training; ++s)
        if (L.need_bwd[s] && L.bwd[s].a.kern == CK_SMALLP) { L.sp_cnt_bwd[s] = c; c += c ? smallp_counters(L.bwd[s].a) : 0; }
      if (training && L.has_pair && L.bwd_pair.a.kern == CK_SMALLP) { L.sp_cnt_pair = c; c += c ? smallp_counters(L.bwd_pair.a) : 0; }
    }
  }
}

static size_t carve_all(vp_pixrefer* h, char* base, size_t cap, std::vector<std::pair<size_t, size_t>>* track = nullptr) {
  Arena ar{base, 0, cap};
  ar.track = track;
// ... 25 lines not shown
    carve_net(h->D, ar, es, true);
    carve_net(h->V, ar, es, true);
    for (Tens& t : h->G.t) if (!t.is_input && t.name != "decoder_1") { t.dz = ar.alloc(t.elems() * es); if (t.hi) t.dz32 = ar.alloc(t.elems() * sizeof(float)); }
    for (Tens& t : h->D.t) if (!t.is_input && t.name != "layer_5") { t.dz = ar.alloc(t.elems() * es); t.dz2 = ar.alloc(t.elems() / 3 * es); }
    for (Net* n : {&h->G, &h->D})
      for (Tens& t : n->t) if (h->bf16 && !t.is_input && !t.has_bn && t.C == 64) t.cs_part = (double*)ar.alloc((size_t)512 * 2 * 64 * sizeof(double));
    for (Tens& t : h->V.t) if (!t.is_input) t.dz = ar.alloc(t.elems() / 2 * es);
    for (const Tens& t : h->V.t) {
      if (t.name == "pool1") h->vpool_code[0] = (unsigned char*)ar.alloc(t.elems() / 2);
      if (t.name == "pool2") h->vpool_code[1] = (unsigned char*)ar.alloc(t.elems() / 2);
    }
    h->n_comp = composite_nblocks(N, H * H);
    h->n_perc = perceptual_nblocks((size_t)N * (H / 4) * (H / 4) * 256, h->bf16);
    h->comp_partial = (double*)ar.alloc((size_t)h->n_comp * 2 * sizeof(double));
    h->perc_partial = (double*)ar.alloc((size_t)h->n_perc * sizeof(double));
  }
  h->zeros = ar.alloc(256);
  h->bn_partial = (double*)ar.alloc((size_t)1024 * 2 * 512 * sizeof(double));
  h->scratch = (char*)ar.alloc(h->scratch_bytes);
  if (d.training) {
    h->bn_partial2 = (double*)ar.alloc((size_t)1024 * 2 * 512 * sizeof(double));
    h->scratch2 = (char*)ar.alloc(h->scratch_bytes);
    h->bn_partial3 = (double*)ar.alloc((size_t)1024 * 2 * 512 * sizeof(double));
    h->scratch3 = (char*)ar.alloc(h->scratch_bytes);
    h->bn_partial4 = (double*)ar.alloc((size_t)1024 * 2 * 512 * sizeof(double));
    h->scratch4 = (char*)ar.alloc(h->scratch_bytes);
  }
  return ar.off + 256;
}

static IgemmArgs pool_fused_view(const IgemmPlan& p) {
  static unsigned char set[16] = {};
  IgemmArgs v = launch_view(p, p.form);
  v.pool_code = set;
  v.pool_src = 1;
  return v;
}

static void init_handle(vp_pixrefer* h, const vp_pixrefer_desc* d) {
  h->d = *d;
  h->bf16 = d->dtype == VP_BF16;
  h->es = h->bf16 ? 2 : 4;
  build_generator(h->G, d->batch, d->height, d->ngf, (!d->training && d->per_sample_bn) ? d->batch : 1);
  size_t smax = 0;
  plan_net(h->G, h->bf16, d->training, d->training, 0, &smax);
  if (d->training) {
    build_discriminator(h->D, d->batch, d->height, d->ndf);
    plan_net(h->D, h->bf16, true, true, d->batch, &smax);
    build_vgg(h->V, d->batch, d->height);
    for (Layer& L : h->V.l) L.g.N = 2 * d->batch;
    plan_net(h->V, h->bf16, true, false, d->batch, &smax, true);
    for (const Layer& L : h->V.l) {
      if (L.scope != "conv1/conv1_2" && L.scope != "conv2/conv2_2") continue;
      const int k = L.scope == "conv2/conv2_2", knob = pool_bwd_fused_knob();
      const IgemmArgs& ba = L.bwd_alt[0].a;
      const bool big = !k || (long long)ba.N * (ba.Hg / 4) * (ba.Wg / 16) >= 4096;
      h->pool_fuse_ok[k] = ((knob == 1 && big) || knob == 2 + k || knob == 4) && h->bf16 && conv_kernel_ok(pool_fused_view(L.bwd_alt[0]), h->bf16);
    }
  }
  h->scratch_bytes = smax + 256;
  h->params_dirty = true;
  h->vgg_dirty = true;
}

static bool valid_desc(const vp_pixrefer_desc* d) {
  if (!d) { set_err("pixrefer descriptor: null"); return false; }
  if (d->batch < 1 || d->height < 256 || d->height % 256 != 0) { set_err("pixrefer descriptor: batch %d / height %d (height must be a multiple of 256)", d->batch, d->height); return false; }
  if (d->ngf < 8 || (d->ngf & (d->ngf - 1)) || d->ndf < 8 || (d->ndf & (d->ndf - 1))) { set_err("pixrefer descriptor: ngf %d / ndf %d must be powers of two >= 8", d->ngf, d->ndf); return false; }
  if (d->ngf > 64 || d->ndf > 64) { set_err("pixrefer descriptor: ngf %d / ndf %d > 64 exceed the batch-norm workspace (512 channels)", d->ngf, d->ndf); return false; }
  if (!d->training && d->per_sample_bn && d->batch > 1024) { set_err("pixrefer descriptor: per-sample batch-norm supports at most 1024 frames per call (got %d)", d->batch); return false; }
  if (d->dtype != VP_F32 && d->dtype != VP_BF16) { set_err("pixrefer descriptor: dtype %d", d->dtype); return false; }
  if ((d->streams != 0 && d->streams != 1 && d->streams != 3 && d->streams != 4) || d->d_backward_fork < 0 || d->d_backward_fork > 3 || d->d_beside_vgg < 0 ||
      d->d_beside_vgg > 2) {
    set_err("pixrefer descriptor: schedule fields streams %d / d_backward_fork %d / d_beside_vgg %d", d->streams, d->d_backward_fork, d->d_beside_vgg);
    return false;
  }
  return true;
}

static void fill_src(const Net& n, const Layer& L, PixSrc& x, int group_n, int sample0, int group0, int es) {
  for (int s = 0; s < 2; ++s) {
    x.ptr[s] = nullptr; x.C[s] = 0; x.aff_a[s] = nullptr; x.aff_b[s] = nullptr;
  }
  for (int s = 0; s < L.nsrc; ++s) {
    const Tens& t = n.t[L.src[s]];
    const void* base = (L.in_act != ACT_NONE) ? t.xa[L.in_act] : t.y;
    x.ptr[s] = (const char*)base + (size_t)sample0 * t.H * t.W * t.C * es;
    x.C[s] = t.C;
  }
  x.act = ACT_NONE;
  x.group_n = group_n;
  (void)group0;
// ... 31 lines not shown
  if (conv_staging(p.a.kern) != CK_PATCH || (p.a.Hg & 1) || (p.a.Wg & 1)) return false;
  int bc, bp;
  igemm_tile(p.cfg, &bc, &bp);
  int th, tw;
  patch_tile_hw(bp, &th, &tw);
  return tw == 16 && th % 2 == 0;
}

static int epi_stat_chunks(const IgemmPlan& p, int batch, int groups) {
  const IgemmArgs& a = p.a;
  const int fam = conv_staging(a.kern);
  if (a.splitk != 1 || fam == CK_SMALLP || fam == CK_S2C64 || batch % groups) return 0;
  int bc, bp;
  igemm_tile(p.cfg, &bc, &bp);
  const int pg = (batch / groups) * a.Hg * a.Wg;
  if (!(fam || groups == 1 || pg % bp == 0)) return 0;
  int pth = 16, ptw = 16;
  patch_tile_hw(bp, &pth, &ptw);
  const int tpg = fam ? (batch / groups) * ((a.Hg + pth - 1) / pth) * ((a.Wg + ptw - 1) / ptw) : (pg + bp - 1) / bp;
  return a.nclass * tpg;
}

static int run_layer_fwd_half(vp_pixrefer* h, Net& n, Layer& L, int half, hipStream_t st, void* pool_out = nullptr, bool pool_only = false,
                              unsigned char* pool_code = nullptr) {
  IgemmArgs a = L.fwd_half.a;
  a.pool_out = pool_out;
  a.pool_only = pool_out && pool_only ? 1 : 0;
  a.pool_code = a.pool_only ? pool_code : nullptr;
  const int nb = a.N;
  fill_src(n, L, a.x, nb, half * nb, 0, h->es);
  a.Wp = n.packed + L.pk_fwd_half * h->es;
  Tens& to = n.t[L.out];
  a.Y = (char*)to.y + (size_t)half * nb * to.H * to.W * to.C * h->es;
  a.bias = n.params + L.b_off;
  a.partial = nullptr;
  a.zeros = h->zeros;
  profile_tag((L.scope + (half ? ":fwd1" : ":fwd0")).c_str());
  VP_HIP_CHECK(launch_igemm(a, h->bf16, L.fwd_half.cfg, st));
  return VP_OK;
}

static bool first_layer_acts_fused(const vp_pixrefer* h, const Net& n, const Layer& L) {
  return first_layer_shape(h->bf16, n, L) && L.fwd.a.kern == CK_CIN8;
}

static int run_layer_fwd(vp_pixrefer* h, Net& n, Layer& L, hipStream_t st, void* pool_out = nullptr, int ss = 0) {
  IgemmArgs a = L.fwd.a;
  a.pool_out = pool_out;
  fill_src(n, L, a.x, n.batch / n.groups, 0, 0, h->es);
  a.Wp = n.packed + L.pk_fwd * h->es;
  Tens& to = n.t[L.out];
  a.Y = L.tapgemm ? L.tap_S : to.y;
  a.bias = L.has_bn || L.tapgemm ? nullptr : n.params + L.b_off;
  a.partial = (float*)scratch_of(h, ss);
  a.zeros = h->zeros;
  if (a.kern == CK_SMALLP) {
    SmallPArgs sp;
    memset(&sp, 0, sizeof(sp));
    a.sp_cnt = L.sp_cnt_fwd;
    sp.g = a;
    for (int c = 0; c < 4; ++c) sp.tap_mask[c] = a.sp_mask[c];
    sp.slab = a.partial; sp.cnt = a.sp_cnt; sp.part = bnp_of(h, ss);
    sp.mode = L.has_bn ? SP_FWD_BN : SP_PLAIN;
    sp.hi = to.hi ? 1 : 0;
    if (L.has_bn) {
      sp.gamma = n.params + L.gamma_off; sp.beta = n.params + L.beta_off;
      sp.aff_a = to.bn.a; sp.aff_b = to.bn.b; sp.mu = to.bn.mu; sp.rstd = to.bn.rstd;
      sp.out_lrelu = to.need_act[ACT_LRELU] ? to.xa[ACT_LRELU] : nullptr;
      sp.out_relu = to.need_act[ACT_RELU] ? to.xa[ACT_RELU] : nullptr;
      sp.eps = 1e-5f;
    }
    profile_tag((L.scope + ":fwd").c_str());
    VP_HIP_CHECK(launch_smallp_fused(sp, h->bf16, st));
    if (!L.has_bn && (to.need_act[ACT_LRELU] || to.need_act[ACT_RELU]))
      VP_HIP_CHECK(launch_act_apply(to.y, nullptr, nullptr, to.C, (n.batch / n.groups) * to.H * to.W, (size_t)to.N * to.H * to.W,
                                    to.xa[ACT_LRELU], to.xa[ACT_RELU], h->bf16, st));
    return VP_OK;
  }
  bool fused_stats = false;
  int stat_chunks = 0;
  if (L.has_bn && a.kern == CK_DC256 && n.groups == 1) {
    stat_chunks = 2 * conv_dc256_grid(a);
    a.bn_part = bnp_of(h, ss); a.bn_tpg = 1 << 30; a.bn_nchunk = stat_chunks;
    fused_stats = true;
  } else if (L.has_bn && a.kern == CK_S2C64) {
// ... 109 lines not shown
  }
  auto try_bst = [&](IgemmArgs& a, const IgemmPlan& p, Tens& ts, int which, bool last) {
    if (!h->bst_on || !last || !ts.has_bn || ts.hi || ts.producer < 0 || ts.is_input) return;
    const int groups = (gpass || alt) ? 1 : n.groups;
    if ((nb / groups) * ts.H * ts.W <= 2048) return;
    if (a.y_f32 || a.ldY % 8 || a.Cout % 8 || a.ldY != ts.C) return;
    if (h->bst_on < 2 && (a.split_c || conv_staging(a.kern) == CK_PATCH || (L.tapgemm && gpass))) return;
    if (a.kern != CK_IGEMM && a.kern != CK_PATCH4 && !(a.kern == CK_PATCH2 && a.x.C[1] == 0)) return;
    const int chunks = epi_stat_chunks(p, nb, groups);
    if (chunks <= 0 || chunks > (gpass ? ts.pbg_cap : ts.pb_cap)) return;
    double* part = gpass ? ts.bn.pbg : ts.bn.pb;
    const void* y = (const char*)ts.y + (size_t)sample0 * ts.H * ts.W * ts.C * es;
    if (which == 0) { a.bn_part = part; a.bst_y = y; }
    else { a.bn_part2 = part; a.bst_y2 = y; }
    a.bn_tpg = chunks / a.nclass; a.bn_nchunk = chunks;
    (gpass ? ts.bst_chunks_g : ts.bst_chunks) = chunks;
    h->bst_count++;
  };
  const bool pair_sp = L.has_pair && L.bwd_pair.a.kern == CK_SMALLP;
  const bool pair_sp_ok = pair_sp && n.t[L.src[0]].has_bn && n.t[L.src[0]].dz_writes + 1 == n.t[L.src[0]].n_bwd_consumers &&
                          n.t[L.src[1]].dz_writes + 1 < n.t[L.src[1]].n_bwd_consumers;
  if (L.has_pair && (parts & 6) == 6 && !alt && !gpass && (!pair_sp || pair_sp_ok)) {
    Tens &t0 = n.t[L.src[0]], &t1 = n.t[L.src[1]];
    IgemmArgs a = L.bwd_pair.a;
    if (pair_sp) {
      set_single_src(a.x, dy, L.g.CoutT, nullptr, nullptr, ACT_NONE, 0);
      a.Wp = n.packed + L.pk_bwd_pair * es;
      a.partial = (float*)scratch;
      a.zeros = h->zeros;
      a.ref = (const char*)t0.xa[L.in_act] + (size_t)sample0 * t0.H * t0.W * t0.C * es;
      a.ref2 = (const char*)t1.xa[L.in_act] + (size_t)sample0 * t1.H * t1.W * t1.C * es;
      a.ref_act = L.in_act;
      a.ref_group_n = group_n;
      a.Y = t0.hi ? t0.dz32 : t0.dz; a.accumulate = t0.dz_written ? 1 : 0;
      a.Y2 = t1.hi ? t1.dz32 : t1.dz; a.accumulate2 = t1.dz_written ? 1 : 0; a.y2_f32 = t1.hi ? 1 : 0;
      t0.dz_written = t1.dz_written = true;
      t0.dz_writes++; t1.dz_writes++;
      SmallPArgs sp;
      memset(&sp, 0, sizeof(sp));
      a.sp_cnt = L.sp_cnt_pair;
      sp.g = a;
      for (int c = 0; c < 4; ++c) sp.tap_mask[c] = a.sp_mask[c];
      sp.slab = a.partial; sp.cnt = a.sp_cnt; sp.part = bn_partial;
      const Layer& Lp = n.l[t0.producer];
      sp.mode = SP_BWD_BN;
      if (t0.hi) { sp.hi = 1; sp.dy_out = t0.dz; }
      sp.bn_y = t0.y; sp.bn_mu = t0.bn.mu; sp.bn_rstd = t0.bn.rstd; sp.bn_gamma = n.params + Lp.gamma_off;
      sp.c1 = t0.bn.c1; sp.c2 = t0.bn.c2;
      sp.dgamma = n.grads + Lp.gamma_off; sp.dbeta = n.grads + Lp.beta_off; sp.dbias_zero = n.grads + Lp.b_off;
      t0.bn_bwd_done = true;
      profile_tag((L.scope + ":bwd").c_str());
      VP_HIP_CHECK(launch_smallp_fused(sp, h->bf16, st));
      return VP_OK;
    }
    set_single_src(a.x, dy, L.g.CoutT, nullptr, nullptr, ACT_NONE, 0);
    a.Wp = n.packed + L.pk_bwd_pair * es;
    a.partial = (float*)scratch;
    a.Y = t0.dz; a.accumulate = t0.dz_written ? 1 : 0;
    a.Y2 = t1.dz; a.accumulate2 = t1.dz_written ? 1 : 0;
    t0.dz_written = t1.dz_written = true;
    t0.dz_writes++; t1.dz_writes++;
    a.ref = (const char*)t0.xa[L.in_act] + (size_t)sample0 * t0.H * t0.W * t0.C * es;
    a.ref2 = (const char*)t1.xa[L.in_act] + (size_t)sample0 * t1.H * t1.W * t1.C * es;
    a.ref_act = L.in_act;
    a.ref_group_n = group_n;
    a.zeros = h->zeros;
    try_bst(a, L.bwd_pair, t0, 0, t0.dz_writes == t0.n_bwd_consumers);
    try_bst(a, L.bwd_pair, t1, 1, t1.dz_writes == t1.n_bwd_consumers);
    profile_tag((L.scope + ":bwd").c_str());
    VP_HIP_CHECK(launch_igemm(a, h->bf16, L.bwd_pair.cfg, st));
    return VP_OK;
  }
  for (int s = 0; s < L.nsrc; ++s) {
    if (!(parts & (2 << s))) continue;
    if (!L.need_bwd[s]) continue;
    Tens& ts = n.t[L.src[s]];
    IgemmArgs a = alt ? L.bwd_alt[s].a : L.bwd[s].a;
    set_single_src(a.x, dy, L.g.CoutT, nullptr, nullptr, ACT_NONE, 0);
    a.Wp = n.packed + (alt ? L.pk_bwd_alt[s] : L.pk_bwd[s]) * es;
    a.partial = (float*)scratch;
    if (ts.is_input) {
      a.Y = (n.groups == 3) ? h->d_din : h->d_vin;
      a.accumulate = 0;
    } else {
      a.Y = gpass ? ts.dz2 : ts.dz;
      if (ts.hi) {
        if (gpass || alt || a.kern != CK_SMALLP) { set_err("%s: float32 few-pixel tensor %s reached by a launch that is not the few-pixel kernel", L.scope.c_str(), ts.name.c_str()); return VP_ERR_STATE; }
        a.Y = ts.dz32; a.y_f32 = 1;
      }
      bool& written = gpass ? ts.dz2_written : ts.dz_written;
      a.accumulate = written ? 1 : 0;
      written = true;
      if (!gpass) {
        ts.dz_writes++;
      }
      a.ref = (const char*)ts.xa[L.in_act] + (size_t)sample0 * ts.H * ts.W * ts.C * es;
      a.ref_act = L.in_act;
      a.ref_group_n = group_n;
    }
    a.zeros = h->zeros;
    profile_tag((L.scope + (alt ? ":bwdG" : ":bwd")).c_str());
    if (a.kern == CK_SMALLP && !alt) {
      SmallPArgs sp;
      memset(&sp, 0, sizeof(sp));
      a.sp_cnt = L.sp_cnt_bwd[s];
      sp.g = a;
      for (int c = 0; c < 4; ++c) sp.tap_mask[c] = a.sp_mask[c];
      sp.slab = a.partial; sp.cnt = a.sp_cnt; sp.part = bn_partial;
      const bool last = !ts.is_input && !gpass && ts.has_bn && ts.producer >= 0 && ts.dz_writes == ts.n_bwd_consumers && n.groups == 1;
      if (ts.hi && !last && ts.dz_writes == ts.n_bwd_consumers) { set_err("%s: float32 tensor %s needs its batch-norm backward in the launch", L.scope.c_str(), ts.name.c_str()); return VP_ERR_STATE; }
      if (last) {
        const Layer& Lp = n.l[ts.producer];
        sp.mode = SP_BWD_BN;
        if (ts.hi) { sp.hi = 1; sp.dy_out = ts.dz; sp.g.y_f32 = 0; }
        sp.bn_y = ts.y; sp.bn_mu = ts.bn.mu; sp.bn_rstd = ts.bn.rstd; sp.bn_gamma = n.params + Lp.gamma_off;
        sp.c1 = ts.bn.c1; sp.c2 = ts.bn.c2;
        sp.dgamma = n.grads + Lp.gamma_off; sp.dbeta = n.grads + Lp.beta_off; sp.dbias_zero = n.grads + Lp.b_off;
        ts.bn_bwd_done = true;
      } else {
        sp.mode = SP_PLAIN;
      }
      VP_HIP_CHECK(launch_smallp_fused(sp, h->bf16, st));
      continue;
    }
    if (L.tapgemm && h->bf16 && cout1_knob() > 0 && !ts.is_input && !ts.hi && !a.accumulate && L.in_act == ACT_LRELU && L.g.ks == 4 && L.g.stride == 1) {
      const int groups = (gpass || alt) ? 1 : n.groups;
      Cout1Args c;
      memset(&c, 0, sizeof(c));
      c.dy = dy; c.ld_dy = L.g.CoutT;
      c.w = n.params + L.w_off;
      c.ref = a.ref; c.ref_act = a.ref_act;
// ... 136 lines not shown
  char* const base = reinterpret_cast<char*>((uintptr_t)1 << 40);
  carve_all(h, base, need, &regs);
  int rc = VP_OK;
  auto fail = [&](const char* fmt, auto... args) { if (rc == VP_OK) { set_err(fmt, args...); rc = VP_ERR_STATE; } };
  size_t prev_end = 0;
  for (size_t i = 0; i < regs.size(); ++i) {
    if (regs[i].first % 256) fail("region %zu at %zu: not 256-byte aligned", i, regs[i].first);
    if (regs[i].first < prev_end) fail("region %zu at %zu overlaps the previous one (ends %zu)", i, regs[i].first, prev_end);
    prev_end = regs[i].first + regs[i].second;
  }
  if (prev_end + 256 > need + 256 || prev_end > need) fail("carved %zu bytes of a %zu-byte workspace", prev_end, need);
  auto region_of = [&](const void* p, size_t bytes, const char* what) {
    if (!p) { fail("%s: null", what); return; }
    const size_t off = (size_t)((const char*)p - base);
    for (const auto& r : regs)
      if (off >= r.first && off + bytes <= r.first + r.second) return;
    fail("%s: [%zu, +%zu) is not inside a carved region", what, off, bytes);
  };
  const int es = h->es;
  for (Net* n : {&h->G, &h->D, &h->V}) {
    if (n->t.empty()) continue;
    for (const Tens& t : n->t) {
      const std::string nm = t.name;
      if (t.name == "decoder_1" || t.name == "layer_5") continue;
      region_of(t.y, t.elems() * (t.hi ? 4 : es), (nm + ".y").c_str());
      for (int k = 1; k < 3; ++k) if (t.need_act[k]) region_of(t.xa[k], t.elems() * es, (nm + ".xa").c_str());
      if (t.has_bn) {
        const size_t gc = (size_t)n->groups * t.C * sizeof(float);
        for (const float* p : {t.bn.a, t.bn.b, t.bn.mu, t.bn.rstd, t.bn.c1, t.bn.c2, t.bn.c1g, t.bn.c2g}) region_of(p, gc, (nm + ".bn").c_str());
        if (d->training && t.pb_cap) region_of(t.bn.pb, (size_t)n->groups * t.pb_cap * 2 * t.C * sizeof(double), (nm + ".bn.pb").c_str());
        if (d->training && t.pbg_cap) region_of(t.bn.pbg, (size_t)t.pbg_cap * 2 * t.C * sizeof(double), (nm + ".bn.pbg").c_str());
        if ((size_t)n->groups * t.C > (size_t)1024 * 512) fail("%s: %d groups x %d channels exceed the batch-norm partial rows", nm.c_str(), n->groups, t.C);
      }
      if (t.cs_part) region_of(t.cs_part, (size_t)512 * 2 * 64 * sizeof(double), (nm + ".cs_part").c_str());
      if (d->training && !t.is_input) {
        const size_t div = n == &h->V ? 2 : 1;
        region_of(t.dz, t.elems() / div * es, (nm + ".dz").c_str());
        if (t.hi) region_of(t.dz32, t.elems() * 4, (nm + ".dz32").c_str());
        if (n == &h->D) region_of(t.dz2, t.elems() / 3 * es, (nm + ".dz2").c_str());
      }
    }
    region_of(n->packed, n->packed_elems * es, "packed weights");
    region_of(n->d_descs, n->descs.size() * sizeof(PackDesc), "pack descriptors");
    for (const PackDesc& p : n->descs) {
      const size_t pe = (size_t)p.nclass * p.Kpad * p.rows_pad;
      if (p.dst_off + pe > n->packed_elems) fail("pack block [%zu, +%zu) outside the %zu-element packed arena", p.dst_off, pe, n->packed_elems);
      if (p.src_off >= n->nparams) fail("pack source %zu outside the %zu-float parameter arena", p.src_off, n->nparams);
    }
    size_t pend = 0;
    for (const ParamInfo& p : n->manifest) {
      size_t cnt = 1;
      for (int i = 0; i < 4; ++i) cnt *= (size_t)p.shape[i];
      if (p.off != pend) fail("parameter %s at %zu: arena not contiguous (expected %zu)", p.name.c_str(), p.off, pend);
      pend = p.off + cnt;
    }
    if (pend != n->nparams) fail("parameter manifest covers %zu of %zu floats", pend, n->nparams);
    for (const Layer& L : n->l) {
      auto plan_ok = [&](const IgemmPlan& p, const char* what) {
        if (p.partial_bytes > h->scratch_bytes) fail("%s %s: split-K slab %zu > scratch %zu", L.scope.c_str(), what, p.partial_bytes, h->scratch_bytes);
        if (p.a.splitk < 1 || p.a.CoutPad < p.a.Cout) fail("%s %s: splitk %d CoutPad %d", L.scope.c_str(), what, p.a.splitk, p.a.CoutPad);
        if (!conv_kernel_ok(launch_view(p, p.form), h->bf16))
          fail("%s %s: the launch is outside the preconditions of its kernel %s", L.scope.c_str(), what, conv_kernel_name(p.a.kern));
      };
      plan_ok(L.fwd, "fwd");
      if (L.has_fwd_half) plan_ok(L.fwd_half, "fwd_half");
      if (d->training && L.has_pair) plan_ok(L.bwd_pair, "bwd_pair");
      if (d->training)
        for (int s2 = 0; s2 < L.nsrc; ++s2) if (L.need_bwd[s2]) { plan_ok(L.bwd[s2], "bwd"); if (n == &h->D || n == &h->V) plan_ok(L.bwd_alt[s2], "bwd_alt"); }
      if (d->training && n != &h->V && L.wg.partial_bytes > h->scratch_bytes) fail("%s wgrad: slab %zu > scratch %zu", L.scope.c_str(), L.wg.partial_bytes, h->scratch_bytes);
      if (L.tapgemm) { region_of(L.tap_S, (size_t)L.g.N * L.g.Hin * L.g.Win * 16 * 4, "tap_S"); region_of(L.tap_dyS, (size_t)L.g.N * L.g.Hin * L.g.Win * 16 * es, "tap_dyS"); }
    }
  }
  const size_t px = (size_t)d->batch * d->height * d->height;
  region_of(h->gin, px * 8 * es, "gin"); region_of(h->gfg, px * 8 * es, "gfg");
  region_of(h->y4, px * 4 * 4, "y4"); region_of(h->o4, px * 4 * 4, "o4");
  region_of(h->outputs, px * 3 * 4, "outputs"); region_of(h->outputs_fg, px * 3 * 4, "outputs_fg");
  region_of(h->scratch, h->scratch_bytes, "scratch"); region_of(h->bn_partial, (size_t)1024 * 2 * 512 * 8, "bn_partial");
  if (d->training) {
    const int hd = d->height / 8 - 2;
    const size_t M = (size_t)d->batch * hd * hd;
    region_of(h->din, 3 * px * 8 * es, "din"); region_of(h->vin, 2 * px * 8 * es, "vin");
    region_of(h->logits, 3 * M * 4, "logits"); region_of(h->predict, 2 * M * 4, "predict");
    region_of(h->dl_d, 3 * M * 8 * es, "dl_d"); region_of(h->dl_g, M * 8 * es, "dl_g");
    region_of(h->d_din, px * 8 * es, "d_din"); region_of(h->d_vin, px * 8 * es, "d_vin"); region_of(h->dy4, px * 8 * es, "dy4");
    for (const Tens& t : h->V.t) {
      if (t.name == "pool1") region_of(h->vpool_code[0], t.elems() / 2, "pool1 codes");
      if (t.name == "pool2") region_of(h->vpool_code[1], t.elems() / 2, "pool2 codes");
    }
    for (const Layer& L : h->V.l) {
      const int k = L.scope == "conv2/conv2_2";
      if ((L.scope != "conv1/conv1_2" && !k) || !h->pool_fuse_ok[k]) continue;
      const Tens& tp = h->V.t[L.out + 1];
      if (tp.name != (k ? "pool2" : "pool1") || tp.H * 2 != h->V.t[L.out].H || tp.C != h->V.t[L.out].C) fail("%s: the tensor behind it is not its 2x2 pool", L.scope.c_str());
      if (L.bwd_alt[0].a.kern != CK_C64 || !conv_kernel_ok(pool_fused_view(L.bwd_alt[0]), h->bf16)) fail("%s bwd_alt: no pooled-source form of kernel %s", L.scope.c_str(), conv_kernel_name(L.bwd_alt[0].a.kern));
      region_of(tp.dz, tp.elems() / 2 * es, (tp.name + ".dz (pooled-source read)").c_str());
      region_of(h->vpool_code[k], tp.elems() / 2, (tp.name + " codes (pooled-source read)").c_str());
    }
    region_of(h->scratch2, h->scratch_bytes, "scratch2"); region_of(h->scratch3, h->scratch_bytes, "scratch3");
    region_of(h->scratch4, h->scratch_bytes, "scratch4"); region_of(h->bn_partial4, (size_t)1024 * 2 * 512 * 8, "bn_partial4");
    region_of(h->bn_partial2, (size_t)1024 * 2 * 512 * 8, "bn_partial2"); region_of(h->bn_partial3, (size_t)1024 * 2 * 512 * 8, "bn_partial3");
  }
  delete h;
  return rc;
}

struct StreamPool {
  int dev = -1;
  hipStream_t side = nullptr, branch = nullptr, branch2 = nullptr;
};
static StreamPool g_pool;
static std::mutex g_pool_mu;

static int pool_streams(bool want_b2, hipStream_t* side, hipStream_t* branch, hipStream_t* branch2) {
  std::lock_guard<std::mutex> lk(g_pool_mu);
  int dev = 0;
  VP_HIP_CHECK(hipGetDevice(&dev));
  if (g_pool.dev >= 0 && g_pool.dev != dev) { set_err("the step executor's streams were created on device %d, this plan is on device %d (one device per process)", g_pool.dev, dev); return VP_ERR_STATE; }
  if (!g_pool.side) {
    int prio_lo = 0, prio_hi = 0;
    (void)hipDeviceGetStreamPriorityRange(&prio_lo, &prio_hi);
    VP_HIP_CHECK(hipStreamCreateWithPriority(&g_pool.side, hipStreamNonBlocking, prio_lo));
    VP_HIP_CHECK(hipStreamCreateWithFlags(&g_pool.branch, hipStreamNonBlocking));
    g_pool.dev = dev;
  }
  if (want_b2 && !g_pool.branch2) VP_HIP_CHECK(hipStreamCreateWithFlags(&g_pool.branch2, hipStreamNonBlocking));
  if (side) *side = g_pool.side;
  if (branch) *branch = g_pool.branch;
  if (branch2) *branch2 = g_pool.branch2;
  return VP_OK;
}
// ... 69 lines not shown
int vp_pixrefer_params_changed(vp_pixrefer_t* h) {
  if (!h) return VP_ERR_ARG;
  h->params_dirty = true;
  h->vgg_dirty = true;
  h->upd_mask = 0;
  return VP_OK;
}

int vp_pixrefer_optimizer_stepped(vp_pixrefer_t* h) {
  if (!h) return VP_ERR_ARG;
  h->params_dirty = true;
  return VP_OK;
}

static int forward_impl(vp_pixrefer_t* h, const float* inputs, const float* fg_inputs, int fg_c, const float* targets, const float* masks, void* stream);

int vp_pixrefer_forward(vp_pixrefer_t* h, const float* inputs, const float* fg_inputs,
                        const float* targets, const float* masks, void* stream) {
  return forward_impl(h, inputs, fg_inputs, 6, targets, masks, stream);
}

int vp_pixrefer_forward_fg3(vp_pixrefer_t* h, const float* inputs, const float* fg_inputs3, const float* targets, void* stream) {
  if (h && h->d.training) { set_err("vp_pixrefer_forward_fg3: inference plans only (the training graph reads fg_inputs[..., 3:], pixrefer.py:297,321)"); return VP_ERR_STATE; }
  return forward_impl(h, inputs, fg_inputs3, 3, targets, nullptr, stream);
}

size_t vp_pixrefer_desc_size(void) { return sizeof(vp_pixrefer_desc); }

static int forward_impl(vp_pixrefer_t* h, const float* inputs, const float* fg_inputs, int fg_c, const float* targets, const float* masks, void* stream) {
  if (!h || !inputs || !fg_inputs || !targets) { set_err("vp_pixrefer_forward: null argument"); return VP_ERR_ARG; }
  const vp_pixrefer_desc& d = h->d;
  if (d.training && !masks) { set_err("vp_pixrefer_forward: masks required when training"); return VP_ERR_ARG; }
  hipStream_t st = (hipStream_t)stream;
  const int N = d.batch, H = d.height, bf = h->bf16;
  int rc;
  if (h->params_dirty) {
    if ((rc = run_pack(h, h->G, st))) return rc;
    if (d.training) {
      if ((rc = run_pack(h, h->D, st))) return rc;
      if (h->vgg_dirty) { if ((rc = run_pack(h, h->V, st))) return rc; h->vgg_dirty = false; }
    }
    h->params_dirty = false;
  }
  h->in_targets = targets; h->in_masks = masks;
  PackInputsArgs pi;
  memset(&pi, 0, sizeof(pi));
  pi.inputs = inputs; pi.fg_inputs = fg_inputs; pi.gin = h->gin; pi.gfg = h->gfg; pi.din = h->din; pi.vin = h->vin;
  pi.N = N; pi.HW = H * H; pi.train = d.training; pi.fg_c = fg_c;
  phase_mark(h, st, 0);
  VP_HIP_CHECK(launch_pack_inputs(pi, bf, st));

  bool split_vgg = d.training && h->overlap && h->ov_on;
  if (split_vgg) for (Layer& L : h->V.l) split_vgg = split_vgg && L.has_fwd_half;
  auto vgg_real_half = [&]() -> int {
    VP_HIP_CHECK(hipEventRecord(h->ev_fork, st));
    VP_HIP_CHECK(hipStreamWaitEvent(h->side, h->ev_fork, 0));
    Net& Vs = h->V;
    for (size_t i = 0; i < Vs.l.size(); ++i) {
      Layer& L = Vs.l[i];
      const bool pooled = L.scope == "conv1/conv1_2" || L.scope == "conv2/conv2_2";
      const bool fuse = pooled && plan_can_pool(L.fwd_half);
      if ((rc = run_layer_fwd_half(h, Vs, L, 0, h->side, fuse ? Vs.t[L.out + 1].y : nullptr, true))) return rc;
      if (pooled && !fuse) {
        const Tens& ti = Vs.t[L.out];
        Tens& tp = Vs.t[L.out + 1];
        VP_HIP_CHECK(launch_maxpool_fwd(ti.y, tp.y, N, ti.H, ti.W, ti.C, bf, h->side));
// ... 204 lines not shown
  h->forked = h->overlap && h->ov_on;
  if (!h->forked) return backward_d_on(h, st, false);
  h->dfork_pending = h->dfork_point;
  if (h->dfork_pending == 0) return fork_d(h, st);
  return VP_OK;
}

void* vp_pixrefer_side_stream(vp_pixrefer_t* h) { return (h && h->overlap) ? (void*)h->side : nullptr; }

int vp_pixrefer_use_streams(vp_pixrefer_t* h, int n) {
  if (!h || (n != 3 && n != 4)) { set_err("vp_pixrefer_use_streams: 3 or 4"); return VP_ERR_ARG; }
  h->use_b2 = (n == 4) && h->overlap;
  return VP_OK;
}

int vp_pixrefer_set_option(vp_pixrefer_t* h, const char* key, int value) {
  if (!h || !key) { set_err("vp_pixrefer_set_option: null argument"); return VP_ERR_ARG; }
  const std::string k(key);
  if (k == "overlap") { h->ov_on = value != 0; return VP_OK; }
  if (k == "d_backward_fork") { h->dfork_point = value < 0 ? 0 : (value > 2 ? 2 : value); return VP_OK; }
  if (k == "d_beside_vgg") { h->dsplit_on = value != 0; return VP_OK; }
  if (k == "store_first_raw") { h->store_first_raw = value != 0; return VP_OK; }
  if (k == "bwd_sums_in_epilogue") { h->bst_on = value < 0 ? 0 : (value > 2 ? 2 : value); return VP_OK; }
  if (k == "vgg_real_fork") { h->vgg_fork_layer = value < 0 ? 0 : value; return VP_OK; }
  set_err("vp_pixrefer_set_option: unknown key %s", key);
  return VP_ERR_ARG;
}

long long vp_pixrefer_counter(vp_pixrefer_t* h, const char* key) {
  if (!h || !key) return -1;
  if (std::string(key) == "bwd_sums_launches") return h->bst_count;
  if (std::string(key) == "pool_codes_written") return h->pool_codes_written ? 1 : 0;
  if (std::string(key) == "pool_bwd_fused") return h->pool_bwd_fused ? 1 : 0;
  return -1;
}

int vp_pixrefer_backward_d_join(vp_pixrefer_t* h, void* stream) {
  if (!h || !h->d.training) { set_err("vp_pixrefer_backward_d_join: needs a training plan"); return VP_ERR_STATE; }
  if (h->forked && h->dfork_pending) {
    const int rc = fork_d(h, (hipStream_t)stream);
    if (rc) return rc;
  }
  if (h->forked) VP_HIP_CHECK(hipStreamWaitEvent((hipStream_t)stream, h->ev_join, 0));
  h->forked = false;
  return VP_OK;
}

static int backward_d_on(vp_pixrefer_t* h, hipStream_t st, bool side) {
  const int N = h->d.batch;
  int rc;
  Net& D = h->D;

  for (Tens& t : D.t) { t.dz_written = false; t.bst_chunks = 0; t.cs_chunks = 0; }
  for (int i = (int)D.l.size() - 1; i >= 0; --i) {
    Layer& L = D.l[i];
    Tens& to = D.t[L.out];
    if (L.has_bn) if ((rc = run_bn_bwd(h, D, L, true, 0, 3 * N, 0, 3, st, side ? 1 : 0))) return rc;
    const bool save = L.need_bwd[0];
    if (i == 0) L.need_bwd[0] = false;
    rc = run_layer_bwd(h, D, L, to.dz, true, false, 0, 3 * N, 0, st, side ? 1 : 0);
    L.need_bwd[0] = save;
    if (rc) return rc;
  }

  return VP_OK;
}
// ... 28 lines not shown
  for (Tens& t : D.t) { t.dz2_written = false; t.bst_chunks_g = 0; }
  for (int i = (int)D.l.size() - 1; i >= 0; --i) {
    Layer& L = D.l[i];
    Tens& to = D.t[L.out];
    if (L.has_bn) if ((rc = run_bn_bwd(h, D, L, false, 2 * N, N, 2, 1, sd, ssd, true))) return rc;
    const void* dy = (i == (int)D.l.size() - 1) ? h->dl_g : to.dz2;
    if ((rc = run_layer_bwd(h, D, L, dy, false, true, 2 * N, N, 2, sd, ssd, true))) return rc;
  }
  if (split_d) VP_HIP_CHECK(hipEventRecord(h->ev_bjoin, h->branch));
  if (h->dfork_pending == 1 && (rc = fork_d(h, st))) return rc;
  for (Tens& t : V.t) t.dz_written = false;
  h->pool_bwd_fused = false;
  h->pool_dz_stale[0] = h->pool_dz_stale[1] = false;
  for (int i = (int)V.l.size() - 1; i >= 0; --i) {
    Layer& L = V.l[i];
    Tens& to = V.t[L.out];
    Tens& ti = V.t[L.src[0]];
    IgemmArgs a = L.bwd_alt[0].a;
    set_single_src(a.x, to.dz, L.g.CoutT, nullptr, nullptr, ACT_NONE, 0);
    const int pk = L.scope == "conv2/conv2_2";
    if ((pk || L.scope == "conv1/conv1_2") && h->pool_dz_stale[pk]) {
      a.x.ptr[0] = V.t[L.out + 1].dz;
      a.pool_code = h->vpool_code[pk];
      a.pool_src = 1;
    }
    a.Wp = V.packed + L.pk_bwd_alt[0] * es;
    a.partial = (float*)h->scratch;
    const bool from_pool = (ti.name == "pool1" || ti.name == "pool2");
    if (ti.is_input) {
      a.Y = h->d_vin;
    } else {
      a.Y = ti.dz;
      if (!from_pool) {
        a.ref = (const char*)ti.y + ti.elems() / 2 * es;
        a.ref_act = ACT_RELU;
      }
    }
    a.zeros = h->zeros;
    profile_tag((L.scope + ":bwd").c_str());
    VP_HIP_CHECK(launch_igemm(a, bf, L.bwd_alt[0].cfg, st));
    if (from_pool) {
      const int ci = L.src[0] - 1;
      Tens& tc = V.t[ci];
      const char* xin = (const char*)tc.y + tc.elems() / 2 * es;
      const int k = ti.name == "pool2";
      if (h->pool_codes_written && h->pool_fuse_ok[k]) {
        h->pool_dz_stale[k] = true;
        h->pool_bwd_fused = true;
      } else if (h->pool_codes_written) VP_HIP_CHECK(launch_maxpool_bwd_code(h->vpool_code[k], ti.dz, tc.dz, N, tc.H, tc.W, tc.C, bf, st));
      else VP_HIP_CHECK(launch_maxpool_bwd(xin, ti.dz, tc.dz, N, tc.H, tc.W, tc.C, bf, st));
    }
  }
  if (split_d) VP_HIP_CHECK(hipStreamWaitEvent(st, h->ev_bjoin, 0));
  if (h->dfork_pending == 2 && (rc = fork_d(h, st))) return rc;
  CompositeArgs ca;
  memset(&ca, 0, sizeof(ca));
  ca.targets = h->in_targets; ca.masks = h->in_masks; ca.o4 = h->o4; ca.outputs = h->outputs;
  ca.d_din = h->d_din; ca.d_vin = h->d_vin; ca.dy4 = h->dy4; ca.N = N; ca.HW = H * H; ca.l1_weight = d.l1_weight;
  VP_HIP_CHECK(launch_composite_bwd(ca, bf, st));
  phase_mark(h, st, 3);
  for (Tens& t : G.t) { t.dz_written = false; t.dz_writes = 0; t.bn_bwd_done = false; t.bst_chunks = 0; t.cs_chunks = 0; }
  }
  const bool split_enc = h->overlap && h->ov_on && l_lo == 0;
  const bool wsplit = h->overlap && h->ov_on;
  bool forked = false, fg_forked = false;
  bool b2_used = false;
  for (int i = l_hi; i >= l_lo; --i) {
// ... 77 lines not shown
  };
  const std::string s(name);
  const int cd = h->bf16 ? VP_BF16 : VP_F32;
  if (s == "Outputs_raw") return ret(h->outputs, N, H, H, 3, VP_F32);
  if (s == "Outputs_FG") return ret(h->outputs_fg, N, H, H, 3, VP_F32);
  if (s == "gen_out4") return ret(h->o4, N, H, H, 4, VP_F32);
  if (s == "losses") return ret(h->losses, 8, 1, 1, 1, VP_F32);
  const int hd = H / 8 - 2;
  if (s == "Predict") return ret(h->predict, 2, N, hd, hd, VP_F32);
  if (s == "logits") return ret(h->logits, 3 * N, hd, hd, 1, VP_F32);
  if (s == "d_gen_out4") return ret(h->dy4, N, H, H, 8, cd);
  if (s == "d_din") return ret(h->d_din, N, H, H, 8, cd);
  if (s == "d_vin") return ret(h->d_vin, N, H, H, 8, cd);
  const size_t c = s.find('/');
  if (c == std::string::npos) return VP_ERR_ARG;
  const std::string net = s.substr(0, c);
  std::string rest = s.substr(c + 1);
  Net* n = net == "g" ? &h->G : net == "d" ? &h->D : net == "v" ? &h->V : nullptr;
  if (!n) return VP_ERR_ARG;
  std::string field;
  const size_t k = rest.find(':');
  if (k != std::string::npos) { field = rest.substr(k + 1); rest = rest.substr(0, k); }
  for (Tens& t : n->t) {
    if (t.name != rest) continue;
    if (field.empty() && !h->store_first_raw && t.producer >= 0 && first_layer_acts_fused(h, *n, n->l[t.producer])) {
      set_err("vp_pixrefer_tensor: the raw output of %s is not stored (its kernel writes the consumers' activations); vp_pixrefer_set_option(h, \"store_first_raw\", 1) before the forward pass", s.c_str());
      return VP_ERR_STATE;
    }
    if (field.empty() && n == &h->V && h->pool_codes_written && (t.name == "conv1/conv1_2" || t.name == "conv2/conv2_2")) {
      set_err("vp_pixrefer_tensor: the full-resolution output of %s is not stored (the step keeps its 2x2 max pool and the pool's arg-max codes); vp_pixrefer_set_option(h, \"store_first_raw\", 1) before the forward pass", s.c_str());
      return VP_ERR_STATE;
    }
    if (field.empty()) return ret(t.y, t.N, t.H, t.W, t.is_f32 ? (t.name == "decoder_1" ? 4 : 1) : t.C, (t.is_f32 || t.hi) ? VP_F32 : cd);
    if (field == "dz32") return t.hi ? ret(t.dz32, t.N, t.H, t.W, t.C, VP_F32) : VP_ERR_ARG;
    if (field == "dy" && n == &h->V && (t.name == "conv1/conv1_2" || t.name == "conv2/conv2_2") && h->pool_dz_stale[t.name == "conv2/conv2_2"]) {
      const int k = t.name == "conv2/conv2_2";
      const Tens& tp = n->t[(&t - n->t.data()) + 1];
      VP_HIP_CHECK(hipDeviceSynchronize());
      VP_HIP_CHECK(launch_maxpool_bwd_code(h->vpool_code[k], tp.dz, t.dz, t.N / 2, t.H, t.W, t.C, h->bf16, nullptr));
      VP_HIP_CHECK(hipDeviceSynchronize());
      h->pool_dz_stale[k] = false;
    }
    if (field == "dy") return ret(t.dz, n == &h->V ? t.N / 2 : t.N, t.H, t.W, t.C, cd);
    if (!t.has_bn) return VP_ERR_ARG;
    if (field == "scale") return ret(t.bn.a, n->groups, t.C, 1, 1, VP_F32);
    if (field == "shift") return ret(t.bn.b, n->groups, t.C, 1, 1, VP_F32);
    if (field == "mean") return ret(t.bn.mu, n->groups, t.C, 1, 1, VP_F32);
    if (field == "rstd") return ret(t.bn.rstd, n->groups, t.C, 1, 1, VP_F32);
    return VP_ERR_ARG;
  }
  return VP_ERR_ARG;
}

int vp_pixrefer_fetch(vp_pixrefer_t* h, int what, void* dst, void* stream) {
  if (!h || !dst || what < 0 || what > 3) { set_err("vp_pixrefer_fetch: bad argument"); return VP_ERR_ARG; }
  FetchArgs f;
  memset(&f, 0, sizeof(f));
  f.raw3 = h->outputs; f.fg3 = h->outputs_fg; f.o4 = h->o4; f.dst = dst;
  f.npix = (size_t)h->d.batch * h->d.height * h->d.height;
  f.mode = what;
  if (what == 3 && h->d.training) {
    VP_HIP_CHECK(hipMemcpyAsync(dst, h->outputs_fg, f.npix * 3 * sizeof(float), hipMemcpyDeviceToDevice, (hipStream_t)stream));
    return VP_OK;
  }
  VP_HIP_CHECK(launch_fetch(f, (hipStream_t)stream));
  return VP_OK;
// ... 26 lines not shown
```

### voicepuppet_amd/engine.py

```python
import ctypes
import os

import numpy as np
import torch

from . import _lib
from ._lib import VP_BF16, VP_F32, PixReferDesc


def _ptr(t):
  return ctypes.c_void_p(t.data_ptr()) if t is not None else ctypes.c_void_p(0)


def _stream():
  return ctypes.c_void_p(torch.cuda.current_stream().cuda_stream)


def manifest(desc, which):
  L = _lib.lib()
  out = []
  name = ctypes.create_string_buffer(256)
  off = ctypes.c_size_t()
  nd = ctypes.c_int()
  shp = (ctypes.c_int64 * 4)()
  i = 0
  while L.vp_pixrefer_param_info(ctypes.byref(desc), which, i, name, 256, ctypes.byref(off), ctypes.byref(nd), shp) == 0:
    out.append((name.value.decode(), int(off.value), tuple(int(shp[k]) for k in range(nd.value))))
    i += 1
  return out


class PixReferEngine:

  def __init__(self, batch, height, ngf=64, ndf=64, dtype="bf16", training=True, l1_weight=500.0, gan_weight=1.0,
               device=None, per_sample_bn=False, streams=0, d_backward_fork=0, d_beside_vgg=0):
    if not torch.cuda.is_available():
      raise RuntimeError("PixReferEngine needs an MI355X (no CPU fallback)")
    self.L = _lib.lib()
    self.device = torch.device(device if device is not None else "cuda:%d" % torch.cuda.current_device())
    self.desc = PixReferDesc(batch, height, ngf, ndf, VP_BF16 if dtype == "bf16" else VP_F32, 1 if training else 0,
# ... 163 lines not shown
        return lambda sp: _lib.check(self.L.vp_pixrefer_update_bucket(self.h, which, bucket, _ptr(m), _ptr(v), t, lr, beta1, 0.999, 1e-8, sp),
                                     "vp_pixrefer_update_bucket")
      ex.begin_step()
      _lib.check(self.L.vp_pixrefer_backward_d_fork(self.h, _stream()), "vp_pixrefer_backward_d_fork")
      d_early = not self.dp_own_stream
      for stage, (lo, hi) in enumerate(self.grad_buckets_g()):
        self.backward_g_stage(stage)
        if stage == 0 and d_early:
          ex.start(self.grads_d, then=update(1, 0), name="discriminator")
        ex.start(self.grads_g[lo:hi], then=update(0, stage), name="generator stage %d" % stage)
      _lib.check(self.L.vp_pixrefer_backward_d_join(self.h, _stream()), "vp_pixrefer_backward_d_join")
      if not d_early:
        ex.start(self.grads_d, then=update(1, 0), name="discriminator")
      ex.finish()
      return
    self.adam_step(lr, beta1)

  def adam_step(self, lr, beta1=0.5, beta2=0.999, eps=1e-8):
    self.t_d += 1
    self.t_g += 1
    for key, p, g, t in (("d", self.params_d, self.grads_d, self.t_d), ("g", self.params_g, self.grads_g, self.t_g)):
      m, v = self.adam[key]
      _lib.check(self.L.vp_adam_tf(_ptr(p), _ptr(g), _ptr(m), _ptr(v), p.numel(), t, lr, beta1, beta2, eps, _stream()),
                 "vp_adam_tf")
    _lib.check(self.L.vp_pixrefer_optimizer_stepped(self.h))

  def tensor(self, name):
    p = ctypes.c_void_p()
    shp = (ctypes.c_int64 * 4)()
    dt = ctypes.c_int()
    _lib.check(self.L.vp_pixrefer_tensor(self.h, name.encode(), ctypes.byref(p), shp, ctypes.byref(dt)),
               "vp_pixrefer_tensor(%s)" % name)
    shape = tuple(int(s) for s in shp)
    tdt = torch.bfloat16 if dt.value == VP_BF16 else torch.float32
    nbytes = int(np.prod(shape)) * (2 if dt.value == VP_BF16 else 4)
    off = p.value - self.workspace.data_ptr()
    assert 0 <= off and off + nbytes <= self.workspace.numel(), name
    return self.workspace[off:off + nbytes].view(tdt).view(shape)

  FETCH = {"Outputs": 0, "Outputs_u8": 1, "Alphas": 2, "Outputs_FG": 3}

  def fetch(self, name):
    n, hgt = self.desc.batch, self.desc.height
    out = torch.empty((n, hgt, hgt, 3), dtype=torch.uint8 if name == "Outputs_u8" else torch.float32, device=self.device)
    _lib.check(self.L.vp_pixrefer_fetch(self.h, self.FETCH[name], _ptr(out), _stream()), "vp_pixrefer_fetch(%s)" % name)
    return out

  def profile(self, on):
    self.L.vp_profile_enable(int(on))
    self.set_option("overlap", 0 if on else 1)

  def set_option(self, key, value):
    _lib.check(self.L.vp_pixrefer_set_option(self.h, key.encode(), int(value)), "vp_pixrefer_set_option(%s)" % key)

  def phase_ms(self):
    buf = (ctypes.c_float * 12)()
    n = self.L.vp_pixrefer_phase_ms(self.h, buf, 12)
    return [float(buf[i]) for i in range(n)]

  def profile_collect(self):
    import json
    n = self.L.vp_profile_collect(None, 0)
    buf = ctypes.create_string_buffer(int(n) + 16)
    self.L.vp_profile_collect(buf, len(buf))
    return json.loads(buf.value.decode())

  def losses(self):
    l = self.tensor("losses").view(-1).float().cpu().numpy()
# ... 3 lines not shown
```

Measured before the change: 4659 frames/s.

## Store 2-bit ReLU sign codes for VGG activations and read them in backward-data

VGG trunk convolutions that write ReLU outputs now also emit a packed 2-bit sign code per element. The matching backward-data kernels read these codes in place of the full bf16 reference activation to build the ReLU mask. The aim is to cut the memory traffic of the backward pass, since the codes are an eighth the size of the bf16 reference. In exchange the forward pass writes an extra array, more kernel template variants are compiled, and new workspace regions and plan consistency checks are added.

```diff
diff --git a/include/vp_hip.h b/include/vp_hip.h
--- a/include/vp_hip.h
+++ b/include/vp_hip.h
@@ -9,7 +9,7 @@
 #endif
 
 enum vp_status { VP_OK = 0, VP_ERR_ARG = -1, VP_ERR_HIP = -2, VP_ERR_WORKSPACE = -3, VP_ERR_STATE = -4 };
-enum vp_dtype { VP_F32 = 0, VP_BF16 = 1 };
+enum vp_dtype { VP_F32 = 0, VP_BF16 = 1, VP_U8 = 2 };
 enum vp_act { VP_ACT_NONE = 0, VP_ACT_LRELU = 1, VP_ACT_RELU = 2, VP_ACT_TANH = 3, VP_ACT_SIGMOID = 4, VP_ACT_RELU6 = 5, VP_ACT_LEAKY = 6 };
 
 int vp_version(void);
@@ -67,6 +67,8 @@
 int vp_pixrefer_use_streams(vp_pixrefer_t* h, int n);
 int vp_pixrefer_set_option(vp_pixrefer_t* h, const char* key, int value);
 long long vp_pixrefer_counter(vp_pixrefer_t* h, const char* key);
+unsigned vp_sign_code_encode8(const uint16_t bits[8]);
+float vp_sign_code_grad(uint16_t code, int e, int act);
 int vp_pixrefer_fetch(vp_pixrefer_t* h, int what, void* dst, void* stream);
 int vp_pixrefer_backward_g_stages(void);
 int vp_pixrefer_backward_g_stage(vp_pixrefer_t* h, int stage, void* stream);
@@ -108,6 +110,9 @@
 size_t vp_conv3x3_c64_bwd_data_pooled_workspace_bytes(const vp_conv_desc* d);
 int vp_conv3x3_c64_bwd_data_pooled(const vp_conv_desc* d, const void* dy_pool, const unsigned char* code, const float* w, const void* ref,
                                    void* dx, void* workspace, int fused, void* stream);
+size_t vp_conv_bwd_data_act_workspace_bytes(const vp_conv_desc* d);
+int vp_conv_bwd_data_act(const vp_conv_desc* d, const void* dy, const float* w, const void* ref, const void* code, int ref_act, int accumulate,
+                         void* dx, void* workspace, void* stream);
 int vp_conv_bwd_weight(const vp_conv_desc* d, const void* x, const float* in_scale, const float* in_shift,
                        const void* dy, float* dw, void* workspace, void* stream);
 
diff --git a/voicepuppet_amd/_lib.py b/voicepuppet_amd/_lib.py
--- a/voicepuppet_amd/_lib.py
+++ b/voicepuppet_amd/_lib.py
@@ -4,7 +4,7 @@
 _HERE = os.path.dirname(os.path.abspath(__file__))
 LIB_PATH = os.environ.get("VP_LIB", os.path.join(_HERE, "libvp_hip.so"))
 
-VP_F32, VP_BF16 = 0, 1
+VP_F32, VP_BF16, VP_U8 = 0, 1, 2
 ACT_NONE, ACT_LRELU, ACT_RELU, ACT_TANH, ACT_SIGMOID = 0, 1, 2, 3, 4
 
 
@@ -180,6 +180,10 @@
     "vp_conv_bwd_weight": (ctypes.c_int, [ctypes.POINTER(ConvDesc), _P, _P, _P, _P, _P, _P, _P]),
     "vp_conv3x3_c64_bwd_data_pooled_workspace_bytes": (ctypes.c_size_t, [ctypes.POINTER(ConvDesc)]),
     "vp_conv3x3_c64_bwd_data_pooled": (ctypes.c_int, [ctypes.POINTER(ConvDesc), _P, _P, _P, _P, _P, _P, ctypes.c_int, _P]),
+    "vp_conv_bwd_data_act_workspace_bytes": (ctypes.c_size_t, [ctypes.POINTER(ConvDesc)]),
+    "vp_conv_bwd_data_act": (ctypes.c_int, [ctypes.POINTER(ConvDesc), _P, _P, _P, _P, ctypes.c_int, ctypes.c_int, _P, _P, _P]),
+    "vp_sign_code_encode8": (ctypes.c_uint, [ctypes.POINTER(ctypes.c_uint16)]),
+    "vp_sign_code_grad": (ctypes.c_float, [ctypes.c_uint16, ctypes.c_int, ctypes.c_int]),
     "vp_bn_workspace_bytes": (ctypes.c_size_t, [ctypes.c_int, ctypes.c_int, ctypes.c_int]),
     "vp_bn_stats": (ctypes.c_int, [_P, ctypes.c_int, ctypes.c_int, ctypes.c_int, _P, _P, ctypes.c_float, _P, _P, _P, _P, _P, _P]),
     "vp_logmel_workspace_bytes": (ctypes.c_size_t, [ctypes.POINTER(LogMelDesc)]),
diff --git a/voicepuppet_amd/csrc/conv_args.h b/voicepuppet_amd/csrc/conv_args.h
--- a/voicepuppet_amd/csrc/conv_args.h
+++ b/voicepuppet_amd/csrc/conv_args.h
@@ -90,6 +90,8 @@
   unsigned* sp_cnt;
   unsigned short sp_mask[4];
   int sp_npt, sp_lcpt;
+  const unsigned short* ref_code;
+  unsigned short* code_out;
 };
 
 struct WgradArgs {
diff --git a/voicepuppet_amd/csrc/conv_c64.hip b/voicepuppet_amd/csrc/conv_c64.hip
--- a/voicepuppet_amd/csrc/conv_c64.hip
+++ b/voicepuppet_amd/csrc/conv_c64.hip
@@ -2,6 +2,7 @@
 #include "igemm_device.h"
 #include "launch.h"
 #include "patch_device.h"
+#include "sign_code.h"
 
 #ifndef C64_LA
 #define C64_LA 2
@@ -66,12 +67,14 @@
   return (unsigned)__builtin_amdgcn_update_dpp(0, (int)v, 0xB1, 0xF, 0xF, true);
 }
 
-template <int NCH, int TPW, int NW, bool REF, bool RELU, bool POOL, bool STORE, bool CODE = false, bool PSRC = false>
+template <int NCH, int TPW, int NW, bool REF, bool RELU, bool POOL, bool STORE, bool CODE = false, bool PSRC = false, bool RCODE = false, bool WCODE = false>
 __global__ __launch_bounds__(NW * 64, 2) void conv_c64_kernel(const IgemmArgs a, const int ntiles) {
   static_assert(!POOL || (RELU && !REF), "the packed max pool compares relu outputs");
   static_assert(!CODE || (POOL && !STORE), "pool codes stand in for the full-resolution store");
   static_assert(!PSRC || (REF && NW % NCH == 0 && PH % (NW / NCH) == 0), "pooled source: backward-data, whole waves per channel chunk");
   static_assert((NCH == 2 && TPW == 2) || (NCH == 4 && TPW == 1), "36 NCH TPW <= 144 weight registers");
+  static_assert(!RCODE || REF, "sign codes stand in for the reference");
+  static_assert(!WCODE || (RELU && STORE && !POOL), "sign codes of a stored relu output");
   constexpr int JP = PPAD / (16 * NW);
   constexpr int CW = 16 * TPW;
   constexpr int COUT = CW * NW, CIN = 32 * NCH;
@@ -151,7 +154,7 @@
   bf16* Yp = reinterpret_cast<bf16*>(a.Y);
   bf16* Pp = reinterpret_cast<bf16*>(a.pool_out);
   constexpr int NSTY = TH * 16 * CB / 1024 / NW;
-  constexpr int NST = (STORE ? NSTY : 0) + (POOL ? TH / 2 : 0) + (CODE ? TH / 2 : 0);
+  constexpr int NST = (STORE ? NSTY * (WCODE ? 2 : 1) : 0) + (POOL ? TH / 2 : 0) + (CODE ? TH / 2 : 0);
 
   const int G = gridDim.x;
   int bt = blockIdx.x;
@@ -220,8 +223,16 @@
     const int n = t / tpi, rem = t - n * tpi;
     const int y0 = (rem / tiles_x) * TH, x0 = (rem % tiles_x) * TW;
     const size_t off00 = ((size_t)(n * a.Hof + y0) * a.Wof + x0 + fi) * COUT + c0;
-    unsigned rz[TH][NV / 2];
-    if constexpr (REF) {
+    unsigned rz[RCODE ? 1 : TH][NV / 2];
+    unsigned rc[TH];
+    if constexpr (RCODE) {
+#pragma unroll
+      for (int r = 0; r < TH; ++r) {
+        const size_t o = off00 + (size_t)r * a.Wof * COUT;
+        if constexpr (NV == 8) rc[r] = a.ref_code[o >> 3];
+        else rc[r] = reinterpret_cast<const unsigned char*>(a.ref_code)[o >> 2];
+      }
+    } else if constexpr (REF) {
 #pragma unroll
       for (int r = 0; r < TH; ++r) {
         if constexpr (NV == 8) {
@@ -308,7 +319,8 @@
       for (int e = 0; e < NV / 2; ++e) {
         unsigned o = Elem<bf16>::pack2(acc[r][(2 * e) >> 2][(2 * e) & 3], acc[r][(2 * e + 1) >> 2][(2 * e + 1) & 3]);
         if constexpr (RELU) o = pk_max_i16(o, 0u);
-        if constexpr (REF) o = pk_mul_lo_u16(o, pk_min_u16(pk_max_i16(rz[r][e], 0u), 0x00010001u));
+        if constexpr (RCODE) o = pk_mul_lo_u16(o, sign_code_relu_pk(rc[r], e));
+        else if constexpr (REF) o = pk_mul_lo_u16(o, pk_min_u16(pk_max_i16(rz[r][e], 0u), 0x00010001u));
         pk[r][e] = o;
       }
     }
@@ -334,6 +346,8 @@
           unsigned* yp = reinterpret_cast<unsigned*>(Yp + ((size_t)(n * a.Hof + y0 + row) * a.Wof + x0 + px) * COUT + sl * 8);
           __builtin_nontemporal_store(o.x, yp); __builtin_nontemporal_store(o.y, yp + 1);
           __builtin_nontemporal_store(o.z, yp + 2); __builtin_nontemporal_store(o.w, yp + 3);
+          if constexpr (WCODE)
+            a.code_out[(((size_t)(n * a.Hof + y0 + row) * a.Wof + x0 + px) * COUT + sl * 8) >> 3] = (unsigned short)sign_code_encode_piece(o.x, o.y, o.z, o.w);
         }
       }
     }
@@ -376,11 +390,13 @@
   if ((a.Cin != 64 && a.Cin != 128) || a.x.C[0] != a.Cin || (a.Cout != 64 && a.Cout != 128)) return false;
   if (a.CoutPad != a.Cout || a.ldY != a.Cout || !a.rowperm || a.splitk != 1) return false;
   if (a.Hg % TH || a.Wg % TW || a.Hin != a.Hg || a.Win != a.Wg || a.Hof != a.Hg || a.Wof != a.Wg) return false;
-  if ((a.out_act != ACT_NONE && a.out_act != ACT_RELU) || (a.ref && (a.ref_act != ACT_RELU || a.out_act != ACT_NONE || a.pool_out))) return false;
+  const bool ref = a.ref || a.ref_code;
+  if ((a.ref && a.ref_code) || (a.out_act != ACT_NONE && a.out_act != ACT_RELU) || (ref && (a.ref_act != ACT_RELU || a.out_act != ACT_NONE || a.pool_out))) return false;
+  if (a.code_out && (ref || a.out_act != ACT_RELU || a.pool_out)) return false;
   if (a.pool_out && (a.out_act != ACT_RELU || (a.Hg & 1))) return false;
   if (a.pool_only && !a.pool_out) return false;
   if (a.pool_code && !a.pool_only && !a.pool_src) return false;
-  if (a.pool_src && (!a.ref || !a.pool_code || a.Cin != a.Cout)) return false;
+  if (a.pool_src && (!ref || !a.pool_code || a.Cin != a.Cout)) return false;
   if (a.bn_part || a.accumulate || a.y_f32 || a.ref_a || a.split_c || a.x.aff_a[0] || a.x.act != ACT_NONE) return false;
   if (a.p_dhs != a.p_dws || a.p_dhf != a.p_dwf || a.p_dhf != (a.p_dhs > 0 ? -1 : 1)) return false;
   return (size_t)a.N * a.Hin * a.Win * a.Cin * 2 < 0x70000000ull;
@@ -390,10 +406,13 @@
 static hipError_t launch_c64_t(const IgemmArgs& a, hipStream_t st) {
   const int ntiles = a.N * (a.Hg / TH) * (a.Wg / TW);
   void (*kern)(const IgemmArgs, const int);
-  if (a.ref && a.pool_src) {
-    if constexpr (16 * TPW * NW == 32 * NCH) kern = conv_c64_kernel<NCH, TPW, NW, true, false, false, true, false, true>;
+  if ((a.ref || a.ref_code) && a.pool_src) {
+    if constexpr (16 * TPW * NW == 32 * NCH) kern = a.ref_code ? conv_c64_kernel<NCH, TPW, NW, true, false, false, true, false, true, true>
+                                                                : conv_c64_kernel<NCH, TPW, NW, true, false, false, true, false, true>;
     else return hipErrorInvalidValue;
-  } else if (a.ref) kern = conv_c64_kernel<NCH, TPW, NW, true, false, false, true>;
+  } else if (a.ref_code) kern = conv_c64_kernel<NCH, TPW, NW, true, false, false, true, false, false, true>;
+  else if (a.ref) kern = conv_c64_kernel<NCH, TPW, NW, true, false, false, true>;
+  else if (a.code_out) kern = conv_c64_kernel<NCH, TPW, NW, false, true, false, true, false, false, false, true>;
   else if (a.pool_out && a.pool_code) kern = conv_c64_kernel<NCH, TPW, NW, false, true, true, false, true>;
   else if (a.pool_out) kern = a.pool_only ? conv_c64_kernel<NCH, TPW, NW, false, true, true, false> : conv_c64_kernel<NCH, TPW, NW, false, true, true, true>;
   else kern = a.out_act == ACT_RELU ? conv_c64_kernel<NCH, TPW, NW, false, true, false, true> : conv_c64_kernel<NCH, TPW, NW, false, false, false, true>;
diff --git a/voicepuppet_amd/csrc/conv_kernels.hip b/voicepuppet_amd/csrc/conv_kernels.hip
--- a/voicepuppet_amd/csrc/conv_kernels.hip
+++ b/voicepuppet_amd/csrc/conv_kernels.hip
@@ -1117,6 +1117,8 @@
 
 bool conv_kernel_ok(const IgemmArgs& a, int is_bf16) {
   if (a.pool_src && a.kern != CK_C64) return false;
+  if (a.ref_code && (a.ref || a.kern != CK_C64)) return false;
+  if (a.code_out && a.kern != CK_C64 && a.kern != CK_CIN8) return false;
   switch (a.kern) {
     case CK_IGEMM: case CK_PATCH: case CK_PATCH2: case CK_SMALLP: return true;
     case CK_S2C64: return conv_s2c64_eligible(a, is_bf16);
diff --git a/voicepuppet_amd/csrc/conv_ops.h b/voicepuppet_amd/csrc/conv_ops.h
--- a/voicepuppet_amd/csrc/conv_ops.h
+++ b/voicepuppet_amd/csrc/conv_ops.h
@@ -64,6 +64,8 @@
 struct LaunchForm {
   bool bias = false, ref = false, xa_lrelu = false, xa_relu = false, x_affine = false;
   bool stats = false;
+  bool ref_code = false;
+  bool code_out = false;
   int x_act = 0, ref_act = 0;
 };
 
@@ -116,6 +118,7 @@
 inline int& patch4_knob() { static int v = 1; return v; }
 inline int& c64_knob() { static int v = 1; return v; }
 inline int& pool_bwd_fused_knob() { static int v = 1; return v; }
+inline int& sign_codes_knob() { static int v = 1; return v; }
 inline int& cout1_knob() { static int v = 256; return v; }
 inline int& wgrad1_rows_knob() { static int v = 512; return v; }
 inline int& dc64_knob() { static int v = 1; return v; }
@@ -292,6 +295,8 @@
   if (v.split_c) v.Y2 = set;
   if (f.bias) v.bias = (const float*)set;
   if (f.ref) { v.ref = set; v.ref_act = f.ref_act; if (v.split_c) v.ref2 = set; }
+  if (f.ref_code) { v.ref_code = (const unsigned short*)set; v.ref_act = f.ref_act; }
+  if (f.code_out) v.code_out = (unsigned short*)set;
   if (f.xa_lrelu) v.xa_lrelu = set;
   if (f.xa_relu) v.xa_relu = set;
   if (f.x_affine) v.x.aff_a[0] = (const float*)set;
diff --git a/voicepuppet_amd/csrc/conv_thin.hip b/voicepuppet_amd/csrc/conv_thin.hip
--- a/voicepuppet_amd/csrc/conv_thin.hip
+++ b/voicepuppet_amd/csrc/conv_thin.hip
@@ -1,12 +1,13 @@
 #include "conv_ops.h"
 #include "igemm_device.h"
 #include "launch.h"
+#include "sign_code.h"
 #include "thin_device.h"
 #include "vp_common.h"
 
 namespace vp {
 
-template <int S, int OUTS>
+template <int S, int OUTS, bool WCODE = false>
 __global__ __launch_bounds__(256) void conv_cin8_kernel(const IgemmArgs a, int lgW, int lgH) {
   const int lane = threadIdx.x & 63;
   const int i = lane & 15, g = lane >> 4;
@@ -82,7 +83,7 @@
       }
     const uint4 plo = Elem<bf16>::pack(lo), phi = Elem<bf16>::pack(hi);
     char* tb = reinterpret_cast<char*>(otile) + (threadIdx.x >> 6) * (16 * 144);
-    auto store_run = [&](void* dst, const uint4& v0, const uint4& v1) {
+    auto store_run = [&](void* dst, const uint4& v0, const uint4& v1, auto wcode) {
       *reinterpret_cast<uint4*>(tb + i * 144 + g * 16) = v0;
       *reinterpret_cast<uint4*>(tb + i * 144 + 64 + g * 16) = v1;
       __builtin_amdgcn_s_waitcnt(0xc07f);
@@ -92,9 +93,14 @@
       bf16* yt = reinterpret_cast<bf16*>(dst) + (size_t)tile * 16 * 64;
       reinterpret_cast<uint4*>(yt)[lane] = q0;
       reinterpret_cast<uint4*>(yt)[64 + lane] = q1;
+      if constexpr (decltype(wcode)::value) {
+        unsigned short* ct = a.code_out + (size_t)tile * (16 * 64 / 8);
+        ct[lane] = (unsigned short)sign_code_encode_piece(q0.x, q0.y, q0.z, q0.w);
+        ct[64 + lane] = (unsigned short)sign_code_encode_piece(q1.x, q1.y, q1.z, q1.w);
+      }
       __builtin_amdgcn_wave_barrier();
     };
-    if constexpr (OUTS & 1) store_run(a.Y, plo, phi);
+    if constexpr (OUTS & 1) store_run(a.Y, plo, phi, std::integral_constant<bool, WCODE>{});
     if constexpr (ACTS) {
       float rl[8], rh[8];
       Elem<bf16>::unpack(plo, rl);
@@ -103,13 +109,13 @@
         float t0[8], t1[8];
 #pragma unroll
         for (int e = 0; e < 8; ++e) { t0[e] = act_apply(ACT_LRELU, rl[e]); t1[e] = act_apply(ACT_LRELU, rh[e]); }
-        store_run(a.xa_lrelu, Elem<bf16>::pack(t0), Elem<bf16>::pack(t1));
+        store_run(a.xa_lrelu, Elem<bf16>::pack(t0), Elem<bf16>::pack(t1), std::false_type{});
       }
       if constexpr (OUTS & 4) {
         float t0[8], t1[8];
 #pragma unroll
         for (int e = 0; e < 8; ++e) { t0[e] = act_apply(ACT_RELU, rl[e]); t1[e] = act_apply(ACT_RELU, rh[e]); }
-        store_run(a.xa_relu, Elem<bf16>::pack(t0), Elem<bf16>::pack(t1));
+        store_run(a.xa_relu, Elem<bf16>::pack(t0), Elem<bf16>::pack(t1), std::false_type{});
       }
     }
   };
@@ -420,7 +426,8 @@
          a.Hof == a.Hg && a.Wof == a.Wg && pow2 && !a.ref && !a.accumulate && !a.y_f32 && !a.bn_part && !a.x.aff_a[0] && a.x.act == ACT_NONE &&
          a.ntaps <= 16 && (a.Kpad == 96 || a.Kpad == 128) && (size_t)a.N * a.Hin * a.Win * 16 < 0x70000000ull &&
          (((long long)a.N * a.Hg * a.Wg) & 15) == 0 && (a.out_act == ACT_NONE || a.out_act == ACT_RELU) &&
-         (a.Kpad == 128 || !(a.xa_lrelu || a.xa_relu)) && !(a.xa_relu && !a.xa_lrelu);
+         (a.Kpad == 128 || !(a.xa_lrelu || a.xa_relu)) && !(a.xa_relu && !a.xa_lrelu) &&
+         !a.ref_code && (!a.code_out || (a.Y && !a.xa_lrelu && !a.xa_relu));
 }
 
 bool conv_cout8_eligible(const IgemmArgs& a, int is_bf16) {
@@ -469,9 +476,10 @@
   const ThinGrid g = thin_grid(a, 3);
   const int outs = (a.Y ? 1 : 0) | (a.xa_lrelu ? 2 : 0) | (a.xa_relu ? 4 : 0);
   void (*kern)(const IgemmArgs, int, int) = nullptr;
-  if (a.Kpad == 96) kern = outs == 1 ? conv_cin8_kernel<3, 1> : nullptr;
+  if (a.code_out && outs != 1) return hipErrorInvalidValue;
+  if (a.Kpad == 96) kern = outs == 1 ? (a.code_out ? conv_cin8_kernel<3, 1, true> : conv_cin8_kernel<3, 1>) : nullptr;
   else switch (outs) {
-    case 1: kern = conv_cin8_kernel<4, 1>; break;
+    case 1: kern = a.code_out ? conv_cin8_kernel<4, 1, true> : conv_cin8_kernel<4, 1>; break;
     case 2: kern = conv_cin8_kernel<4, 2>; break;
     case 3: kern = conv_cin8_kernel<4, 3>; break;
     case 6: kern = conv_cin8_kernel<4, 6>; break;
diff --git a/voicepuppet_amd/csrc/ops_api.hip b/voicepuppet_amd/csrc/ops_api.hip
--- a/voicepuppet_amd/csrc/ops_api.hip
+++ b/voicepuppet_amd/csrc/ops_api.hip
@@ -6,6 +6,7 @@
 #include "errors.h"
 #include "audio_args.h"
 #include "launch.h"
+#include "sign_code.h"
 #include "vp_common.h"
 
 using namespace vp;
@@ -53,6 +54,14 @@
 }
 
 extern "C" void vp_phase_marks_enable(int on);
+
+unsigned vp_sign_code_encode8(const uint16_t bits[8]) {
+  if (!bits) return 0u;
+  const unsigned c = vp::sign_code_encode8(bits);
+  auto pk = [&](int i) { return (unsigned)bits[2 * i] | ((unsigned)bits[2 * i + 1] << 16); };
+  return vp::sign_code_encode_piece(pk(0), pk(1), pk(2), pk(3)) == c ? c : ~0u;
+}
+float vp_sign_code_grad(uint16_t code, int e, int act) { return e < 0 || e > 7 ? 0.f : vp::sign_code_grad(code, e, act); }
 
 int vp_tune(const char* key, int value) {
   if (!key) return VP_ERR_ARG;
@@ -66,6 +75,7 @@
   if (k == "c64") { c64_knob() = value; return VP_OK; }
   if (k == "dc64") { dc64_knob() = value; return VP_OK; }
   if (k == "pool_bwd_fused") { pool_bwd_fused_knob() = value < 0 || value > 4 ? 1 : value; return VP_OK; }
+  if (k == "sign_codes") { sign_codes_knob() = value < 0 || value > 2 ? 1 : value; return VP_OK; }
   if (k == "cout1_wgrad_rows" && value > 0) { wgrad1_rows_knob() = value; return VP_OK; }
   if (k == "cout1_bwd") { cout1_knob() = value < 0 ? 256 : value; return VP_OK; }
   if (k == "s2c64") { s2c64_knob() = value; return VP_OK; }
@@ -177,6 +187,42 @@
   return VP_OK;
 }
 
+static bool bwd_act_desc_ok(const vp_conv_desc* d) { return conv_desc_ok(d) && d->cout >= 8 && !(d->cout & (d->cout - 1)); }
+
+size_t vp_conv_bwd_data_act_workspace_bytes(const vp_conv_desc* d) { return bwd_act_desc_ok(d) ? vp_conv_workspace_bytes(d) : 0; }
+
+int vp_conv_bwd_data_act(const vp_conv_desc* d, const void* dy, const float* w, const void* ref, const void* code, int ref_act, int accumulate,
+                         void* dx, void* workspace, void* stream) {
+  if (!bwd_act_desc_ok(d) || !dy || !w || !dx || !workspace || (ref != nullptr) == (code != nullptr) || (ref_act != ACT_LRELU && ref_act != ACT_RELU) ||
+      (accumulate != 0 && accumulate != 1) || (code && (d->dtype != VP_BF16 || d->cin % 8))) {
+    set_err("vp_conv_bwd_data_act: bad argument (one of ref / code, ref_act leaky ReLU or ReLU, accumulate 0 / 1; codes: bf16, channels a multiple of 8)");
+    return VP_ERR_ARG;
+  }
+  const int bf = d->dtype == VP_BF16, es = bf ? 2 : 4;
+  hipStream_t st = (hipStream_t)stream;
+  const ConvGeomX g = geom_of(d);
+  IgemmPlan p = plan_bwd_data(g, 0, 0, d->cin, d->cin, d->cin, bf);
+  p.a.accumulate = accumulate;
+  LaunchForm f;
+  f.ref = ref != nullptr; f.ref_code = code != nullptr; f.ref_act = ref_act;
+  plan_kernel(p, d->cin, bf, d->cout, 0, FAM_PATCH | FAM_PATCH2, f);
+  if (!conv_kernel_ok(launch_view(p, f), bf)) {
+    set_err("vp_conv_bwd_data_act: the launch is planned on kernel %s, which does not take %s", conv_kernel_name(p.a.kern), code ? "sign codes in this form" : "this form");
+    return VP_ERR_ARG;
+  }
+  char* ws = (char*)workspace;
+  VP_HIP_CHECK(launch_pack_weights_one(p.pack, w, ws, bf, st));
+  IgemmArgs a = p.a;
+  set_single_src(a.x, dy, d->cout, nullptr, nullptr, ACT_NONE, 0);
+  a.Wp = ws;
+  a.partial = (float*)(ws + align256(p.pack_elems * es));
+  a.Y = dx;
+  a.ref = ref; a.ref_code = (const unsigned short*)code; a.ref_act = ref_act; a.ref_group_n = d->n;
+  a.zeros = zero_page(ws, align256(p.pack_elems * es) + p.partial_bytes, st);
+  VP_HIP_CHECK(launch_igemm(a, bf, p.cfg, st));
+  return VP_OK;
+}
+
 static bool pooled_desc_ok(const vp_conv_desc* d) {
   return conv_desc_ok(d) && d->kind == 0 && d->ksize == 3 && d->stride == 1 && d->pad == 1 && d->dtype == VP_BF16 && d->cin == d->cout &&
          (d->cin == 64 || d->cin == 128) && d->h % 4 == 0 && d->w % 16 == 0 && d->h >= 16;
diff --git a/voicepuppet_amd/csrc/plan_pixrefer.hip b/voicepuppet_amd/csrc/plan_pixrefer.hip
--- a/voicepuppet_amd/csrc/plan_pixrefer.hip
+++ b/voicepuppet_amd/csrc/plan_pixrefer.hip
@@ -53,6 +53,8 @@
   void* dz2 = nullptr;
   bool dz2_written = false;
   void* xa[3] = {nullptr, nullptr, nullptr};
+  unsigned short* code = nullptr;
+  bool code_on = false;
   bool need_act[3] = {false, false, false};
   BnBuf bn{};
   int producer = -1;
@@ -133,6 +135,8 @@
   bool pool_fuse_ok[2];
   bool pool_bwd_fused;
   bool pool_dz_stale[2];
+  int sc_launches, sc_ref_launches;
+  unsigned sc_kernels;
   double *comp_partial, *perc_partial, *bn_partial;
   char* scratch;
   char* scratch2;
@@ -461,6 +465,7 @@
     }
     if (!t.is_input) t.y = ar.alloc(t.elems() * (t.hi ? sizeof(float) : (size_t)es));
     for (int k = 1; k < 3; ++k) if (t.need_act[k]) t.xa[k] = ar.alloc(t.elems() * es);
+    if (t.code_on) t.code = (unsigned short*)ar.alloc(t.elems() / 4);
     if (t.has_bn) {
       const size_t gc = (size_t)n.groups * t.C * sizeof(float);
       t.bn.a = (float*)ar.alloc(gc); t.bn.b = (float*)ar.alloc(gc);
@@ -552,6 +557,7 @@
 static IgemmArgs pool_fused_view(const IgemmPlan& p) {
   static unsigned char set[16] = {};
   IgemmArgs v = launch_view(p, p.form);
+  if (!v.ref && !v.ref_code) { v.ref = set; v.ref_act = ACT_RELU; }
   v.pool_code = set;
   v.pool_src = 1;
   return v;
@@ -578,6 +584,29 @@
       h->pool_fuse_ok[k] = ((knob == 1 && big) || knob == 2 + k || knob == 4) && h->bf16 && conv_kernel_ok(pool_fused_view(L.bwd_alt[0]), h->bf16);
     }
   }
+  if (d->training && h->bf16 && sign_codes_knob()) {
+    for (Layer& L : h->V.l) {
+      if (!L.need_bwd[0]) continue;
+      Tens& ts = h->V.t[L.src[0]];
+      IgemmPlan& rd = L.bwd_alt[0];
+      if (ts.is_input || ts.producer < 0 || !rd.form.ref || rd.form.ref_act != ACT_RELU) continue;
+      if (sign_codes_knob() != 2 && ts.C != 64) continue;
+      Layer& P = h->V.l[ts.producer];
+      LaunchForm fr = rd.form, fw = P.fwd.form, fh = P.fwd_half.form;
+      fr.ref = false; fr.ref_code = true;
+      fw.code_out = fh.code_out = true;
+      auto same = [&](const IgemmPlan& p, const LaunchForm& f) { const IgemmArgs v = launch_view(p, f); return pick_conv_kernel(v, 1) == p.a.kern && conv_kernel_ok(v, 1); };
+      if (!same(rd, fr) || !same(P.fwd, fw) || !P.has_fwd_half || !same(P.fwd_half, fh)) continue;
+      const int pk = L.scope == "conv2/conv2_2";
+      if ((pk || L.scope == "conv1/conv1_2") && h->pool_fuse_ok[pk]) {
+        IgemmArgs v = pool_fused_view(rd);
+        v.ref = nullptr; v.ref_code = (const unsigned short*)h->pool_fuse_ok;
+        if (!conv_kernel_ok(v, 1)) continue;
+      }
+      rd.form = fr; P.fwd.form = fw; P.fwd_half.form = fh;
+      ts.code_on = true;
+    }
+  }
   h->scratch_bytes = smax + 256;
   h->params_dirty = true;
   h->vgg_dirty = true;
@@ -675,6 +704,7 @@
   a.Wp = n.packed + L.pk_fwd_half * h->es;
   Tens& to = n.t[L.out];
   a.Y = (char*)to.y + (size_t)half * nb * to.H * to.W * to.C * h->es;
+  if (L.fwd_half.form.code_out && half == 1) a.code_out = to.code + (size_t)half * nb * to.H * to.W * to.C / 8;
   a.bias = n.params + L.b_off;
   a.partial = nullptr;
   a.zeros = h->zeros;
@@ -694,6 +724,7 @@
   a.Wp = n.packed + L.pk_fwd * h->es;
   Tens& to = n.t[L.out];
   a.Y = L.tapgemm ? L.tap_S : to.y;
+  if (L.fwd.form.code_out) a.code_out = to.code;
   a.bias = L.has_bn || L.tapgemm ? nullptr : n.params + L.b_off;
   a.partial = (float*)scratch_of(h, ss);
   a.zeros = h->zeros;
@@ -869,6 +900,7 @@
       a.ref2 = (const char*)t1.xa[L.in_act] + (size_t)sample0 * t1.H * t1.W * t1.C * es;
       a.ref_act = L.in_act;
       a.ref_group_n = group_n;
+      h->sc_ref_launches++;
       a.Y = t0.hi ? t0.dz32 : t0.dz; a.accumulate = t0.dz_written ? 1 : 0;
       a.Y2 = t1.hi ? t1.dz32 : t1.dz; a.accumulate2 = t1.dz_written ? 1 : 0; a.y2_f32 = t1.hi ? 1 : 0;
       t0.dz_written = t1.dz_written = true;
@@ -901,6 +933,7 @@
     a.ref2 = (const char*)t1.xa[L.in_act] + (size_t)sample0 * t1.H * t1.W * t1.C * es;
     a.ref_act = L.in_act;
     a.ref_group_n = group_n;
+    h->sc_ref_launches++;
     a.zeros = h->zeros;
     try_bst(a, L.bwd_pair, t0, 0, t0.dz_writes == t0.n_bwd_consumers);
     try_bst(a, L.bwd_pair, t1, 1, t1.dz_writes == t1.n_bwd_consumers);
@@ -934,6 +967,7 @@
       a.ref = (const char*)ts.xa[L.in_act] + (size_t)sample0 * ts.H * ts.W * ts.C * es;
       a.ref_act = L.in_act;
       a.ref_group_n = group_n;
+      h->sc_ref_launches++;
     }
     a.zeros = h->zeros;
     profile_tag((L.scope + (alt ? ":bwdG" : ":bwd")).c_str());
@@ -1136,6 +1170,10 @@
         if (d->training && t.pbg_cap) region_of(t.bn.pbg, (size_t)t.pbg_cap * 2 * t.C * sizeof(double), (nm + ".bn.pbg").c_str());
         if ((size_t)n->groups * t.C > (size_t)1024 * 512) fail("%s: %d groups x %d channels exceed the batch-norm partial rows", nm.c_str(), n->groups, t.C);
       }
+      if (t.code_on) {
+        region_of(t.code, t.elems() / 4, (nm + ".code").c_str());
+        if (!h->bf16 || !d->training || t.C % 8 || t.producer < 0) fail("%s: sign codes outside a bf16 training plan / a channel count %d that is no multiple of 8", nm.c_str(), t.C);
+      }
       if (t.cs_part) region_of(t.cs_part, (size_t)512 * 2 * 64 * sizeof(double), (nm + ".cs_part").c_str());
       if (d->training && !t.is_input) {
         const size_t div = n == &h->V ? 2 : 1;
@@ -1200,6 +1238,21 @@
       region_of(tp.dz, tp.elems() / 2 * es, (tp.name + ".dz (pooled-source read)").c_str());
       region_of(h->vpool_code[k], tp.elems() / 2, (tp.name + " codes (pooled-source read)").c_str());
     }
+    for (const Layer& L : h->V.l) {
+      if (!L.need_bwd[0]) continue;
+      const Tens& ts = h->V.t[L.src[0]];
+      const LaunchForm& fr = L.bwd_alt[0].form;
+      if (fr.ref && fr.ref_code) fail("%s bwd_alt: reference and sign codes", L.scope.c_str());
+      if (fr.ref_code != ts.code_on) fail("%s bwd_alt: reads codes %d, %s has codes %d", L.scope.c_str(), (int)fr.ref_code, ts.name.c_str(), (int)ts.code_on);
+      if (L.bwd[0].form.ref_code) fail("%s bwd: the whole-batch backward plan is not a code reader", L.scope.c_str());
+    }
+    for (const Net* n : {&h->G, &h->D, &h->V})
+      for (const Layer& L : n->l) {
+        const bool on = n->t[L.out].code_on;
+        if (L.fwd.form.code_out != on || (L.has_fwd_half ? L.fwd_half.form.code_out : false) != (on && L.has_fwd_half) || (on && !L.has_fwd_half))
+          fail("%s: code writers (fwd %d, fwd_half %d) do not match the tensor's code array (%d)", L.scope.c_str(), (int)L.fwd.form.code_out, (int)L.fwd_half.form.code_out, (int)on);
+        if (on && n != &h->V) fail("%s: sign codes outside the VGG trunk", L.scope.c_str());
+      }
     region_of(h->scratch2, h->scratch_bytes, "scratch2"); region_of(h->scratch3, h->scratch_bytes, "scratch3");
     region_of(h->scratch4, h->scratch_bytes, "scratch4"); region_of(h->bn_partial4, (size_t)1024 * 2 * 512 * 8, "bn_partial4");
     region_of(h->bn_partial2, (size_t)1024 * 2 * 512 * 8, "bn_partial2"); region_of(h->bn_partial3, (size_t)1024 * 2 * 512 * 8, "bn_partial3");
@@ -1335,6 +1388,7 @@
   const vp_pixrefer_desc& d = h->d;
   if (d.training && !masks) { set_err("vp_pixrefer_forward: masks required when training"); return VP_ERR_ARG; }
   hipStream_t st = (hipStream_t)stream;
+  h->sc_launches = h->sc_ref_launches = 0; h->sc_kernels = 0;
   const int N = d.batch, H = d.height, bf = h->bf16;
   int rc;
   if (h->params_dirty) {
@@ -1605,6 +1659,9 @@
   if (std::string(key) == "bwd_sums_launches") return h->bst_count;
   if (std::string(key) == "pool_codes_written") return h->pool_codes_written ? 1 : 0;
   if (std::string(key) == "pool_bwd_fused") return h->pool_bwd_fused ? 1 : 0;
+  if (std::string(key) == "sign_code_launches") return h->sc_launches;
+  if (std::string(key) == "sign_code_ref_launches") return h->sc_ref_launches;
+  if (std::string(key) == "sign_code_kernels") return h->sc_kernels;
   return -1;
 }
 
@@ -1699,7 +1756,13 @@
     } else {
       a.Y = ti.dz;
       if (!from_pool) {
-        a.ref = (const char*)ti.y + ti.elems() / 2 * es;
+        if (L.bwd_alt[0].form.ref_code) {
+          a.ref_code = ti.code + ti.elems() / 2 / 8;
+          h->sc_launches++; h->sc_kernels |= 1u << conv_staging(a.kern);
+        } else {
+          a.ref = (const char*)ti.y + ti.elems() / 2 * es;
+          h->sc_ref_launches++;
+        }
         a.ref_act = ACT_RELU;
       }
     }
@@ -1843,6 +1906,7 @@
       return VP_ERR_STATE;
     }
     if (field.empty()) return ret(t.y, t.N, t.H, t.W, t.is_f32 ? (t.name == "decoder_1" ? 4 : 1) : t.C, (t.is_f32 || t.hi) ? VP_F32 : cd);
+    if (field == "code") return (n == &h->V && t.code_on) ? ret(t.code, t.N, t.H, t.W, t.C / 4, VP_U8) : VP_ERR_ARG;
     if (field == "dz32") return t.hi ? ret(t.dz32, t.N, t.H, t.W, t.C, VP_F32) : VP_ERR_ARG;
     if (field == "dy" && n == &h->V && (t.name == "conv1/conv1_2" || t.name == "conv2/conv2_2") && h->pool_dz_stale[t.name == "conv2/conv2_2"]) {
       const int k = t.name == "conv2/conv2_2";
diff --git a/voicepuppet_amd/csrc/sign_code.h b/voicepuppet_amd/csrc/sign_code.h
--- /dev/null
+++ b/voicepuppet_amd/csrc/sign_code.h
@@ -0,0 +1,45 @@
+#pragma once
+#include <stdint.h>
+
+#if defined(__HIPCC__) || defined(__CUDACC__)
+#define VP_SC_HD __host__ __device__ inline
+#else
+#define VP_SC_HD inline
+#endif
+
+namespace vp {
+
+enum { SIGN_CODE_ACT_LRELU = 1, SIGN_CODE_ACT_RELU = 2 };
+
+VP_SC_HD unsigned sign_code_of(unsigned b) { return (b & 0x7fffu) == 0 ? 0u : ((b & 0x8000u) ? 2u : 1u); }
+
+VP_SC_HD unsigned sign_code_pair(unsigned w) {
+  const unsigned nz = ((w & 0x7fff7fffu) + 0x7fff7fffu) & 0x80008000u;
+  const unsigned neg = nz & w, pos = nz ^ neg;
+  const unsigned c = (pos >> 15) | (neg >> 14);
+  return (c | (c >> 14)) & 0xfu;
+}
+
+VP_SC_HD unsigned sign_code_encode_piece(unsigned x, unsigned y, unsigned z, unsigned w) {
+  return sign_code_pair(x) | (sign_code_pair(y) << 4) | (sign_code_pair(z) << 8) | (sign_code_pair(w) << 12);
+}
+
+VP_SC_HD unsigned sign_code_encode8(const uint16_t bits[8]) {
+  unsigned c = 0;
+  for (int e = 0; e < 8; ++e) c |= sign_code_of(bits[e]) << (2 * e);
+  return c;
+}
+
+VP_SC_HD float sign_code_grad(unsigned code, int e, int act) {
+  const unsigned c = (code >> (2 * e)) & 3u;
+  if (act == SIGN_CODE_ACT_LRELU) return c == 1u ? 1.0f : (c == 2u ? 0.2f : 0.6f);
+  if (act == SIGN_CODE_ACT_RELU) return c == 1u ? 1.f : 0.f;
+  return 1.f;
+}
+
+VP_SC_HD unsigned sign_code_relu_pk(unsigned code, int p) {
+  const unsigned x = code >> (4 * p);
+  return (x & 1u) | ((x & 4u) << 14);
+}
+
+}
diff --git a/voicepuppet_amd/engine.py b/voicepuppet_amd/engine.py
--- a/voicepuppet_amd/engine.py
+++ b/voicepuppet_amd/engine.py
@@ -5,7 +5,7 @@
 import torch
 
 from . import _lib
-from ._lib import VP_BF16, VP_F32, PixReferDesc
+from ._lib import VP_BF16, VP_F32, VP_U8, PixReferDesc
 
 
 def _ptr(t):
@@ -235,8 +235,8 @@
     _lib.check(self.L.vp_pixrefer_tensor(self.h, name.encode(), ctypes.byref(p), shp, ctypes.byref(dt)),
                "vp_pixrefer_tensor(%s)" % name)
     shape = tuple(int(s) for s in shp)
-    tdt = torch.bfloat16 if dt.value == VP_BF16 else torch.float32
-    nbytes = int(np.prod(shape)) * (2 if dt.value == VP_BF16 else 4)
+    tdt = {VP_BF16: torch.bfloat16, VP_U8: torch.uint8}.get(dt.value, torch.float32)
+    nbytes = int(np.prod(shape)) * {VP_BF16: 2, VP_U8: 1}.get(dt.value, 4)
     off = p.value - self.workspace.data_ptr()
     assert 0 <= off and off + nbytes <= self.workspace.numel(), name
     return self.workspace[off:off + nbytes].view(tdt).view(shape)
```

New measurement: 4657 frames/s. No clear change (-0.0%).
